# basilevh/tcow

Measured on AMD Instinct MI355X. Metric: train clips/sec (T=30, 240x320), higher is better.
Workload: dtype bf16; 1 GPU; TCOW Seeker train step: T=30 240x320 patch16, 12-layer divided space-time ViT (D=768), num_queries=3, causal_attention=1, 1 clip/GPU; clips_per_gpu=1, num_queries=3, parallelism=dp1, optimizer=AdamW lr 1e-4, clip 0.3

## Files before the change

### include/tcow_hip.h

```cpp
#ifndef TCOW_HIP_H
#define TCOW_HIP_H

#ifdef __cplusplus
extern "C" {
#endif

#define TCOW_OK 0
#define TCOW_ERR_INVALID_ARG (-1)
#define TCOW_ERR_LAUNCH (-2)
#define TCOW_ERR_UNSUPPORTED (-3)

#define TCOW_F32 0
#define TCOW_BF16 1
#define TCOW_F32X3 2

#define TCOW_ACT_NONE 0
#define TCOW_ACT_GELU 1
#define TCOW_ACT_DGELU 2
#define TCOW_ACT_GELU_DSAVE 3
#define TCOW_ACT_MUL_AUX 4

#define TCOW_ABI_VERSION 11
int tcow_version(void);
const char* tcow_last_error(void);

typedef struct {
    int M, N, K;
    int dtype;
    const void* A; long lda;
    const void* W; long ldw;
    void* C; long ldc; int out_f32;
    const float* bias;
    const float* row_scale;
    const float* resid; long ldr;
    int act;
    void* aux; long ldaux;
    int tile;
    const float* bias2;
    const float* row_scale2;
} tcow_gemm_args;
int tcow_gemm_nt(void* stream, const tcow_gemm_args* args);

int tcow_prof_gemm_begin(int max_launches);
int tcow_prof_gemm_end(double* total_ms, double* total_flops, long* launches);
int tcow_prof_attn_begin(int max_launches);
int tcow_prof_attn_end(double* ms4, double* flops4, double* bytes4, long* launches4);

long tcow_gemm_tn_workspace_bytes(int M, int N, int K);
int tcow_gemm_tn(void* stream, int dtype, int M, int N, int K, const void* dY, long ldy, const void* X,
                 long ldx, float* dW, long lddw, float* bias_grad, int accumulate, void* workspace,
                 long workspace_bytes);

typedef struct {
    int M, N, K;
    const void* dY; long ldy;
    const void* X; long ldx;
    float* dW; long lddw;
    float* bias_grad;
    int accumulate;
} tcow_tn_problem;
long tcow_gemm_tn_grouped_workspace_bytes(int dtype, int n, const tcow_tn_problem* problems);
int tcow_gemm_tn_grouped(void* stream, int dtype, int n, const tcow_tn_problem* problems, void* workspace, long workspace_bytes);
int tcow_gemm_tn_group_max(void);

typedef struct {
    int M, N, K;
    const float* A; long sai, sak;
    const float* B; long sbj, sbk;
    float* C; long ldc;
    int accumulate;
} tcow_sgemm;
int tcow_sgemm_x3_batched(void* stream, int n, const tcow_sgemm* problems);

int tcow_layernorm_fwd(void* stream, int dtype, int rows, int D, const float* x, long ldx, const float* gamma,
                       const float* beta, float eps, void* y, long ldy, float* mean, float* rstd);
long tcow_layernorm_bwd_workspace_bytes(int D);
int tcow_layernorm_bwd(void* stream, int dtype, int rows, int D, const void* dy, long lddy, const float* x, long ldx,
                       const float* mean, const float* rstd, const float* gamma, const float* dres, long lddres,
                       float* dx, long lddx, float* dgamma, float* dbeta, int accumulate, void* workspace,
                       long workspace_bytes, void* dx_cast, long lddx_cast, const float* cast_row_scale,
                       const float* colsum_row_scale, float* colsum_out);
typedef struct {
    const float* part; int parts, D;
    float* dgamma; float* dbeta; float* colsum_out;
    int accumulate;
} tcow_ln_fold_job;
int tcow_layernorm_bwd_parts(int rows, int with_colsum);
int tcow_layernorm_fold(void* stream, int n, const tcow_ln_fold_job* jobs);

typedef struct {
    int B, T, S;
    int D, heads;
    int causal;
    int dtype;
} tcow_attn_shape;
int tcow_attn_temporal_fwd(void* stream, const tcow_attn_shape* shape, const void* qkv, void* out, float* lse);
int tcow_attn_spatial_fwd(void* stream, const tcow_attn_shape* shape, const void* qkv, void* out, float* lse);
long tcow_attn_bwd_workspace_bytes(const tcow_attn_shape* shape);
int tcow_attn_temporal_bwd(void* stream, const tcow_attn_shape* shape, const void* qkv, const void* out,
                           const void* dout, const float* lse, void* dqkv, void* workspace, long workspace_bytes);
int tcow_attn_spatial_bwd(void* stream, const tcow_attn_shape* shape, const void* qkv, const void* out,
                          const void* dout, const float* lse, void* dqkv, void* workspace, long workspace_bytes);

#define TCOW_STREAM_MAX_FRAMES 1024
int tcow_attn_temporal_cached_fwd(void* stream, const tcow_attn_shape* chunk, int T_total, const int* t0_dev, const void* qkv, void* k_cache,
                                  void* v_cache, void* out);
int tcow_cls_stream(void* stream, int B, int c, int S, int D, float* x, float* cls_cache, const int* t0_dev);

int tcow_im2col(void* stream, int dtype, int B, int T, int H, int W, int P, const float* rgb, const float* query,
                int pretrained_norm, void* out);
int tcow_im2col_channels(void* stream, int dtype, int B, int T, int H, int W, int P, int C, const float* src,
                         int normalise, void* out);
int tcow_gather_frames(void* stream, int elem_bytes, int C, int Tv, int H, int W, int Tc, int h, int w, const void* src,
                       const int* frame_idx, const int* src_y, const int* src_x, void* out);
int tcow_resize_aa(void* stream, int C, int Tv, int H, int W, int Tc, int hc, int wc, int oh, int ow, const float* src, const int* frame_idx,
                   const int* ys, const int* xs, const int* ymin, const int* ysize, const float* wy, int ky, const int* xmin, const int* xsize,
                   const float* wx, int kx, float* out);

long tcow_photometric_workspace_bytes(int Tc);
int tcow_photometric(void* stream, int Tv, int H, int W, int Tc, int y0, int x0, int h, int w, const float* src, const int* frame_idx, int n_ops,
                     const int* ops, float brightness, float contrast, float saturation, float hue, int blur, const float* taps, int gray,
                     float* workspace, long workspace_bytes, float* out);

int tcow_embed_fwd(void* stream, int B, int T, int S, int D, float* x, const float* cls, const float* pos,
                   const float* time_embed);
int tcow_embed_bwd(void* stream, int B, int T, int S, int D, const float* g, float* dpos, float* dtime,
                   int accumulate);
int tcow_cls_merge(void* stream, int B, int T, int S, int D, float* x, int mode, int backward);
int tcow_cls_merge_bwd_cast(void* stream, int dtype, int B, int T, int S, int D, float* x, int mode, void* cast_out, long ldc,
                            const float* cast_scale);

int tcow_unpatchify_pool_fwd(void* stream, int dtype, int BT, int Hp, int Wp, int P, int C, int st, const void* pm,
                             float* pooled);
int tcow_unpatchify_pool_bwd(void* stream, int dtype, int BT, int Hp, int Wp, int P, int C, int st,
                             const float* dpooled, void* dpm);
int tcow_upsample_fwd(void* stream, int B, int T, int C, int h, int w, int st, int bilinear, const float* pooled,
                      float* out);
int tcow_upsample_bwd(void* stream, int B, int T, int C, int h, int w, int st, int bilinear, const float* dout,
                      float* dpooled);
#define TCOW_AMAX_SLOTS 64
int tcow_upsample_bwd_amax(void* stream, int B, int T, int C, int h, int w, int st, const float* dout, float* dpooled,
                           unsigned* amax_bits, int n_slots);
int tcow_flags_fwd(void* stream, int BT, int S, int D, int F, const float* x, const float* Wf, const float* bf,
                   float* flags);

int tcow_scale_unless_one(void* stream, float* x, long n, const float* scale);
int tcow_scale_cast(void* stream, int dtype, long rows, int D, const float* src, long ld_src, const float* row_scale,
                    void* dst, long ld_dst);
int tcow_droppath_rows(void* stream, int depth, int B, int T, int S, const float* u, const float* keep_p, const float* mask0, float* out);
int tcow_cast_transpose(void* stream, int dtype, int N, int K, const float* W, void* Wc, void* Wt);
long tcow_cast_desc_bytes(void);
int tcow_cast_transpose_batched(void* stream, int dtype, const void* table, int n, int total_tiles);

long tcow_adamw_chunk_bytes(void);
int tcow_adamw_clip_step(void* stream, const void* chunks, int n_chunks, float lr, float beta1, float beta2, float eps,
                         float weight_decay, int step, float max_norm, float* scratch);
int tcow_adamw_clip_step_scaled(void* stream, const void* chunks, int n_chunks, float lr, float beta1, float beta2, float eps,
                                float weight_decay, int step, float max_norm, float* scratch, const float* grad_inv_scale);
long tcow_adamw_tile_bytes(void);
int tcow_adamw_clip_step_cast(void* stream, const void* chunks, int n_chunks, const void* flat_chunks, int n_flat, const void* tiles, int n_tiles, float lr, float beta1,
                              float beta2, float eps, float weight_decay, int step, float max_norm, float* scratch, const float* grad_inv_scale);

typedef struct {
    long n_frames, frame_len, frames_per_seq;
    const float* logits;  long logits_seq_stride;
    const float* target;  long target_seq_stride;
    const float* pixel_w;
    const float* frame_w;
    int weighted_aot;
    float aot_loss;
    double topk_frac;
    float loss_weight;
    float* loss;
    float* total;
    float* dlogits;  long dlogits_seq_stride;
    void* ws;  size_t ws_bytes;
    int focal;
} tcow_mask_loss_args;
size_t tcow_mask_loss_workspace_bytes(long n_frames, long frame_len);
size_t tcow_mask_loss_workspace_bytes_for(long n_frames, long frame_len, double topk_frac, float aot_loss);
int tcow_mask_loss(void* stream, const tcow_mask_loss_args* args);
int tcow_mask_loss_batch(void* stream, const tcow_mask_loss_args* args, int n);

int tcow_iou_counts(void* stream, const float* logits, const float* target, long n_frames, long frame_len, int* counts);

int tcow_build_masks(void* stream, int B, int Q, int M, int T, long HW, int query_time, const unsigned char* segm,
                     const unsigned char* div_segm, const int* query_idx, const int* front_idx, const int* cont_idx,
                     float* query_mask, float* target_mask, unsigned char* snitch_occl_by_ptr, int* counts);

int tcow_build_query_masks(void* stream, int B, int Q, int K, int M, int T, long HW, int query_time, const unsigned char* segm,
                           const unsigned char* div_segm, const float* occl_fracs, const float* dag, const long long* sel, float front_thres,
                           float front_half_thres, float outer_thres, float occluded_weight, float zero_weight, float has_weight, int* idx_ws,
                           unsigned char* ids, float* flags, float* sel_occl_fracs, float* frame_w, float* query_mask, float* target_mask,
                           unsigned char* snitch_occl_by_ptr, int* counts);

int tcow_iou_means(void* stream, const int* counts, int n_seq, int C, int T, float* mean, int* count);

size_t tcow_snitch_weights_workspace_bytes(long n_frames, int H, int W);
int tcow_snitch_weights(void* stream, long n_seq, int T, int H, int W, const float* target_ch0, long target_seq_stride,
                        const unsigned char* snitch_occl_by_ptr, const float* frame_w, const int* pos_count, int class_balancing,
                        float hard_negative_factor, float* weights, void* ws, size_t ws_bytes);

#ifdef __cplusplus
}
#endif
#endif
```

### tcow_amd/_lib.py

```python
import ctypes
import os

_HERE = os.path.dirname(os.path.abspath(__file__))
LIB_PATH = os.environ.get('TCOW_LIB') or os.path.join(_HERE, 'libtcow_hip.so')
LIB_PATH_FP16 = os.path.join(_HERE, 'libtcow_hip_fp16.so')

TCOW_F32, TCOW_BF16, TCOW_F32X3 = 0, 1, 2
ACT_NONE, ACT_GELU, ACT_DGELU, ACT_GELU_DSAVE, ACT_MUL_AUX = 0, 1, 2, 3, 4


class TcowError(RuntimeError):
    """Raised when a libtcow_hip entry point returns a non-zero status (message from tcow_last_error)."""


class AttnShape(ctypes.Structure):
    _fields_ = [('B', ctypes.c_int), ('T', ctypes.c_int), ('S', ctypes.c_int), ('D', ctypes.c_int),
                ('heads', ctypes.c_int), ('causal', ctypes.c_int), ('dtype', ctypes.c_int)]


class GemmArgs(ctypes.Structure):
    _fields_ = [('M', ctypes.c_int), ('N', ctypes.c_int), ('K', ctypes.c_int), ('dtype', ctypes.c_int),
                ('A', ctypes.c_void_p), ('lda', ctypes.c_long), ('W', ctypes.c_void_p), ('ldw', ctypes.c_long),
                ('C', ctypes.c_void_p), ('ldc', ctypes.c_long), ('out_f32', ctypes.c_int),
                ('bias', ctypes.c_void_p), ('row_scale', ctypes.c_void_p), ('resid', ctypes.c_void_p),
                ('ldr', ctypes.c_long), ('act', ctypes.c_int), ('aux', ctypes.c_void_p), ('ldaux', ctypes.c_long), ('tile', ctypes.c_int),
                ('bias2', ctypes.c_void_p), ('row_scale2', ctypes.c_void_p)]


class SGemm(ctypes.Structure):
    _fields_ = [('M', ctypes.c_int), ('N', ctypes.c_int), ('K', ctypes.c_int),
                ('A', ctypes.c_void_p), ('sai', ctypes.c_long), ('sak', ctypes.c_long),
                ('B', ctypes.c_void_p), ('sbj', ctypes.c_long), ('sbk', ctypes.c_long),
                ('C', ctypes.c_void_p), ('ldc', ctypes.c_long), ('accumulate', ctypes.c_int)]


class TnProblem(ctypes.Structure):
    _fields_ = [('M', ctypes.c_int), ('N', ctypes.c_int), ('K', ctypes.c_int),
                ('dY', ctypes.c_void_p), ('ldy', ctypes.c_long), ('X', ctypes.c_void_p), ('ldx', ctypes.c_long),
                ('dW', ctypes.c_void_p), ('lddw', ctypes.c_long), ('bias_grad', ctypes.c_void_p), ('accumulate', ctypes.c_int)]


class LnFoldJob(ctypes.Structure):
    _fields_ = [('part', ctypes.c_void_p), ('parts', ctypes.c_int), ('D', ctypes.c_int), ('dgamma', ctypes.c_void_p), ('dbeta', ctypes.c_void_p),
                ('colsum_out', ctypes.c_void_p), ('accumulate', ctypes.c_int)]


class MaskLossArgs(ctypes.Structure):
    _fields_ = [('n_frames', ctypes.c_long), ('frame_len', ctypes.c_long), ('frames_per_seq', ctypes.c_long),
                ('logits', ctypes.c_void_p), ('logits_seq_stride', ctypes.c_long),
                ('target', ctypes.c_void_p), ('target_seq_stride', ctypes.c_long),
                ('pixel_w', ctypes.c_void_p), ('frame_w', ctypes.c_void_p),
                ('weighted_aot', ctypes.c_int), ('aot_loss', ctypes.c_float), ('topk_frac', ctypes.c_double),
                ('loss_weight', ctypes.c_float), ('loss', ctypes.c_void_p), ('total', ctypes.c_void_p),
                ('dlogits', ctypes.c_void_p), ('dlogits_seq_stride', ctypes.c_long),
                ('ws', ctypes.c_void_p), ('ws_bytes', ctypes.c_size_t), ('focal', ctypes.c_int)]


_libs = {}

_vp, _i, _l, _f = ctypes.c_void_p, ctypes.c_int, ctypes.c_long, ctypes.c_float
_ash = ctypes.POINTER(AttnShape)
SIGNATURES = {
    'tcow_version': (_i, []),
    'tcow_last_error': (ctypes.c_char_p, []),
    'tcow_gemm_nt': (_i, [_vp, ctypes.POINTER(GemmArgs)]),
    'tcow_prof_gemm_begin': (_i, [_i]),
    'tcow_prof_gemm_end': (_i, [ctypes.POINTER(ctypes.c_double), ctypes.POINTER(ctypes.c_double), ctypes.POINTER(ctypes.c_long)]),
    'tcow_prof_attn_begin': (_i, [_i]),
    'tcow_prof_attn_end': (_i, [_vp, _vp, _vp, _vp]),
    'tcow_gemm_tn_workspace_bytes': (_l, [_i, _i, _i]),
    'tcow_gemm_tn': (_i, [_vp, _i, _i, _i, _i, _vp, _l, _vp, _l, _vp, _l, _vp, _i, _vp, _l]),
    'tcow_gemm_tn_grouped_workspace_bytes': (_l, [_i, _i, _vp]),
    'tcow_gemm_tn_grouped': (_i, [_vp, _i, _i, _vp, _vp, _l]),
    'tcow_gemm_tn_group_max': (_i, []),
    'tcow_sgemm_x3_batched': (_i, [_vp, _i, _vp]),
    'tcow_layernorm_fwd': (_i, [_vp, _i, _i, _i, _vp, _l, _vp, _vp, _f, _vp, _l, _vp, _vp]),
    'tcow_layernorm_bwd_workspace_bytes': (_l, [_i]),
    'tcow_layernorm_bwd': (_i, [_vp, _i, _i, _i, _vp, _l, _vp, _l, _vp, _vp, _vp, _vp, _l, _vp, _l, _vp, _vp, _i, _vp, _l, _vp, _l, _vp, _vp, _vp]),
    'tcow_layernorm_bwd_parts': (_i, [_i, _i]),
    'tcow_layernorm_fold': (_i, [_vp, _i, _vp]),
    'tcow_attn_temporal_fwd': (_i, [_vp, _ash, _vp, _vp, _vp]),
    'tcow_attn_spatial_fwd': (_i, [_vp, _ash, _vp, _vp, _vp]),
    'tcow_attn_bwd_workspace_bytes': (_l, [_ash]),
    'tcow_attn_temporal_bwd': (_i, [_vp, _ash, _vp, _vp, _vp, _vp, _vp, _vp, _l]),
    'tcow_attn_spatial_bwd': (_i, [_vp, _ash, _vp, _vp, _vp, _vp, _vp, _vp, _l]),
    'tcow_attn_temporal_cached_fwd': (_i, [_vp, _ash, _i, _vp, _vp, _vp, _vp, _vp]),
    'tcow_cls_stream': (_i, [_vp, _i, _i, _i, _i, _vp, _vp, _vp]),
    'tcow_im2col': (_i, [_vp, _i, _i, _i, _i, _i, _i, _vp, _vp, _i, _vp]),
    'tcow_gather_frames': (_i, [_vp, _i, _i, _i, _i, _i, _i, _i, _i, _vp, _vp, _vp, _vp, _vp]),
    'tcow_resize_aa': (_i, [_vp, _i, _i, _i, _i, _i, _i, _i, _i, _i, _vp, _vp, _vp, _vp, _vp, _vp, _vp, _i, _vp, _vp, _vp, _i, _vp]),
    'tcow_photometric_workspace_bytes': (_l, [_i]),
    'tcow_photometric': (_i, [_vp, _i, _i, _i, _i, _i, _i, _i, _i, _vp, _vp, _i, ctypes.POINTER(ctypes.c_int), _f, _f, _f, _f, _i, ctypes.POINTER(ctypes.c_float), _i,
                         _vp, _l, _vp]),
    'tcow_im2col_channels': (_i, [_vp, _i, _i, _i, _i, _i, _i, _i, _vp, _i, _vp]),
    'tcow_embed_fwd': (_i, [_vp, _i, _i, _i, _i, _vp, _vp, _vp, _vp]),
    'tcow_embed_bwd': (_i, [_vp, _i, _i, _i, _i, _vp, _vp, _vp, _i]),
    'tcow_cls_merge': (_i, [_vp, _i, _i, _i, _i, _vp, _i, _i]),
    'tcow_cls_merge_bwd_cast': (_i, [_vp, _i, _i, _i, _i, _i, _vp, _i, _vp, _l, _vp]),
    'tcow_unpatchify_pool_fwd': (_i, [_vp, _i, _i, _i, _i, _i, _i, _i, _vp, _vp]),
    'tcow_unpatchify_pool_bwd': (_i, [_vp, _i, _i, _i, _i, _i, _i, _i, _vp, _vp]),
    'tcow_upsample_fwd': (_i, [_vp, _i, _i, _i, _i, _i, _i, _i, _vp, _vp]),
    'tcow_upsample_bwd': (_i, [_vp, _i, _i, _i, _i, _i, _i, _i, _vp, _vp]),
    'tcow_upsample_bwd_amax': (_i, [_vp, _i, _i, _i, _i, _i, _i, _vp, _vp, _vp, _i]),
    'tcow_flags_fwd': (_i, [_vp, _i, _i, _i, _i, _vp, _vp, _vp, _vp]),
    'tcow_droppath_rows': (_i, [_vp, _i, _i, _i, _i, _vp, _vp, _vp, _vp]),
    'tcow_scale_cast': (_i, [_vp, _i, _l, _i, _vp, _l, _vp, _vp, _l]),
    'tcow_scale_unless_one': (_i, [_vp, _vp, _l, _vp]),
    'tcow_cast_transpose': (_i, [_vp, _i, _i, _i, _vp, _vp, _vp]),
    'tcow_cast_desc_bytes': (_l, []),
    'tcow_cast_transpose_batched': (_i, [_vp, _i, _vp, _i, _i]),
    'tcow_adamw_chunk_bytes': (_l, []),
    'tcow_adamw_clip_step': (_i, [_vp, _vp, _i, _f, _f, _f, _f, _f, _i, _f, _vp]),
    'tcow_adamw_clip_step_scaled': (_i, [_vp, _vp, _i, _f, _f, _f, _f, _f, _i, _f, _vp, _vp]),
    'tcow_adamw_tile_bytes': (_l, []),
    'tcow_adamw_clip_step_cast': (_i, [_vp, _vp, _i, _vp, _i, _vp, _i, _f, _f, _f, _f, _f, _i, _f, _vp, _vp]),
    'tcow_mask_loss_workspace_bytes': (ctypes.c_size_t, [_l, _l]),
    'tcow_mask_loss_workspace_bytes_for': (ctypes.c_size_t, [_l, _l, ctypes.c_double, _f]),
    'tcow_mask_loss': (_i, [_vp, ctypes.POINTER(MaskLossArgs)]),
    'tcow_mask_loss_batch': (_i, [_vp, ctypes.POINTER(MaskLossArgs), _i]),
    'tcow_iou_counts': (_i, [_vp, _vp, _vp, _l, _l, _vp]),
    'tcow_build_masks': (_i, [_vp, _i, _i, _i, _i, _l, _i, _vp, _vp, _vp, _vp, _vp, _vp, _vp, _vp, _vp]),
    'tcow_build_query_masks': (_i, [_vp, _i, _i, _i, _i, _i, _l, _i, _vp, _vp, _vp, _vp, _vp, _f, _f, _f, _f, _f, _f, _vp, _vp, _vp, _vp, _vp, _vp, _vp, _vp, _vp]),
    'tcow_iou_means': (_i, [_vp, _vp, _i, _i, _i, _vp, _vp]),
    'tcow_snitch_weights_workspace_bytes': (ctypes.c_size_t, [_l, _i, _i]),
    'tcow_snitch_weights': (_i, [_vp, _l, _i, _i, _i, _vp, _l, _vp, _vp, _vp, _i, _f, _vp, _vp, ctypes.c_size_t]),
}


ABI_VERSION = 11


def _declare(L, tolerant=False):
    for name, (res, args) in SIGNATURES.items():
        if tolerant and not hasattr(L, name):
            continue
        fn = getattr(L, name)
        fn.restype = res
        fn.argtypes = args



def lib(fmt='bf16'):
    L = _libs.get(fmt)
    if L is None:
        path = LIB_PATH if fmt == 'bf16' else LIB_PATH_FP16
        if not os.path.exists(path):
            raise TcowError(f'{path} not found: build it with `make` (or __graft_entry__.build()); '
                            'the Seeker HIP path has no fallback')
        import torch
        L = ctypes.CDLL(path)
        L.tcow_last_error.restype = ctypes.c_char_p
        L.tcow_version.restype = ctypes.c_int
        if L.tcow_version() != ABI_VERSION and not (fmt == 'bf16' and os.environ.get('TCOW_LIB')):
            raise TcowError(f'{path} reports ABI version {L.tcow_version()}, this host code was written against {ABI_VERSION} (include/tcow_hip.h): rebuild with `make`')
        _declare(L, tolerant=(fmt == 'bf16' and bool(os.environ.get('TCOW_LIB'))))
        _libs[fmt] = L
    return L


def check(rc, what='', L=None):
    if rc != 0:
        raise TcowError(f'{what} failed (status {rc}): {(L or lib()).tcow_last_error().decode()}')
```

### tcow_amd/csrc/gemm_x3.hip

```cpp
#include "gemm_f32.h"

namespace {

constexpr int XT = 128;
constexpr int XK = 32;
constexpr int XP = 80;
constexpr int XPLANE = XT * XP;

typedef __attribute__((ext_vector_type(8))) __bf16 x3_bf16x8;
typedef __attribute__((ext_vector_type(2))) __bf16 x3_bf16x2;
__device__ __forceinline__ uint32_t x3_pack(float a, float b) {
    f32x2 v = {a, b};
    return __builtin_bit_cast(uint32_t, __builtin_convertvector(v, x3_bf16x2));
}
__device__ __forceinline__ void split2(float x0, float x1, uint32_t& h, uint32_t& l) {
    h = x3_pack(x0, x1);
    l = x3_pack(x0 - __builtin_bit_cast(float, h << 16), x1 - __builtin_bit_cast(float, h & 0xffff0000u));
}

enum { LD_ANY = 0, LD_KVEC = 1, LD_RVEC = 2 };

template <int LD>
__device__ __forceinline__ void load_regs(const float* __restrict__ P, long s_row, long s_k, int row0, int nrows, int k0, int K, f32x4 (&v)[4], int tid) {
    if (LD == LD_KVEC) {
        const int kq = k0 + (tid & 7) * 4, r = tid >> 3;
        const int kc = kq < K - 4 ? kq : K - 4;
#pragma unroll
        for (int ps = 0; ps < 4; ++ps) {
            int gr = row0 + r + 32 * ps; gr = gr < nrows ? gr : nrows - 1;
            v[ps] = *reinterpret_cast<const f32x4*>(P + (size_t)gr * s_row + kc);
        }
    } else if (LD == LD_RVEC) {
        const int rq = 4 * ((tid & 7) + 8 * (tid >> 6));
        int gr = row0 + rq; gr = gr < nrows - 4 ? gr : nrows - 4;
#pragma unroll
        for (int ps = 0; ps < 2; ++ps) {
            const int k = k0 + 2 * (((tid >> 3) & 7) + 8 * ps);
            const int kc0 = k < K ? k : K - 1, kc1 = k + 1 < K ? k + 1 : K - 1;
            v[2 * ps] = *reinterpret_cast<const f32x4*>(P + (size_t)kc0 * s_k + gr);
            v[2 * ps + 1] = *reinterpret_cast<const f32x4*>(P + (size_t)kc1 * s_k + gr);
        }
    } else {
        const int iq = tid & 31, kp = tid >> 5;
#pragma unroll
        for (int e = 0; e < 4; ++e) {
            int gr = row0 + iq + 32 * e; gr = gr < nrows ? gr : nrows - 1;
#pragma unroll
            for (int ps = 0; ps < 2; ++ps) {
                const int k = k0 + 2 * (kp + 8 * ps);
                const int kc0 = k < K ? k : K - 1, kc1 = k + 1 < K ? k + 1 : K - 1;
                v[e][2 * ps] = P[(size_t)gr * s_row + (size_t)kc0 * s_k];
                v[e][2 * ps + 1] = P[(size_t)gr * s_row + (size_t)kc1 * s_k];
            }
        }
    }
}

template <int LD>
__device__ __forceinline__ void mask_tail(f32x4 (&v)[4], int k0, int kend, int tid) {
    const f32x4 zero = {0.f, 0.f, 0.f, 0.f};
    if (LD == LD_KVEC) {
        const bool live = k0 + (tid & 7) * 4 < kend;
#pragma unroll
        for (int e = 0; e < 4; ++e) v[e] = live ? v[e] : zero;
    } else if (LD == LD_RVEC) {
#pragma unroll
        for (int ps = 0; ps < 2; ++ps) {
            const int k = k0 + 2 * (((tid >> 3) & 7) + 8 * ps);
            v[2 * ps] = k < kend ? v[2 * ps] : zero;
            v[2 * ps + 1] = k + 1 < kend ? v[2 * ps + 1] : zero;
        }
    } else {
#pragma unroll
        for (int e = 0; e < 4; ++e)
#pragma unroll
            for (int ps = 0; ps < 2; ++ps) {
                const int k = k0 + 2 * ((tid >> 5) + 8 * ps);
                v[e][2 * ps] = k < kend ? v[e][2 * ps] : 0.f; v[e][2 * ps + 1] = k + 1 < kend ? v[e][2 * ps + 1] : 0.f;
            }
    }
}

template <int LD>
__device__ __forceinline__ void store_split(const f32x4 (&v)[4], char* hi_plane, char* lo_plane, int tid) {
    if (LD == LD_KVEC) {
        const int kq = tid & 7, r = tid >> 3;
#pragma unroll
        for (int ps = 0; ps < 4; ++ps) {
            uint2 h, l;
            split2(v[ps][0], v[ps][1], h.x, l.x);
            split2(v[ps][2], v[ps][3], h.y, l.y);
            const int off = (r + 32 * ps) * XP + kq * 8;
            *reinterpret_cast<uint2*>(hi_plane + off) = h;
            *reinterpret_cast<uint2*>(lo_plane + off) = l;
        }
    } else if (LD == LD_RVEC) {
        const int rq = 4 * ((tid & 7) + 8 * (tid >> 6));
#pragma unroll
        for (int ps = 0; ps < 2; ++ps) {
            const int kp = ((tid >> 3) & 7) + 8 * ps;
#pragma unroll
            for (int e = 0; e < 4; ++e) {
                uint32_t h, l;
                split2(v[2 * ps][e], v[2 * ps + 1][e], h, l);
                const int off = (rq + e) * XP + kp * 4;
                *reinterpret_cast<uint32_t*>(hi_plane + off) = h;
                *reinterpret_cast<uint32_t*>(lo_plane + off) = l;
            }
        }
    } else {
        const int iq = tid & 31, kp = tid >> 5;
#pragma unroll
        for (int e = 0; e < 4; ++e)
#pragma unroll
            for (int ps = 0; ps < 2; ++ps) {
                uint32_t h, l;
                split2(v[e][2 * ps], v[e][2 * ps + 1], h, l);
                const int off = (iq + 32 * e) * XP + (kp + 8 * ps) * 4;
                *reinterpret_cast<uint32_t*>(hi_plane + off) = h;
                *reinterpret_cast<uint32_t*>(lo_plane + off) = l;
            }
    }
}

__device__ __forceinline__ int cdiv_dev(int a, int b) { return (a + b - 1) / b; }

__device__ __forceinline__ x3_bf16x8 frag(const char* plane, int row, int ks, int hi) {
    return __builtin_bit_cast(x3_bf16x8, *reinterpret_cast<const uint4*>(plane + row * XP + ks * 32 + hi * 16));
}

template <int LDA, int LDB>
__device__ __forceinline__ void gemm_x3_body(const F32Params& p, const int bid, const int kz, char* smem) {
    char* a_hi = smem; char* a_lo = smem + XPLANE; char* b_hi = smem + 2 * XPLANE; char* b_lo = smem + 3 * XPLANE;
    const int tid = threadIdx.x, lane = tid & 63, wave = tid >> 6;
    const int wm = wave >> 1, wn = wave & 1, l31 = lane & 31, hi = lane >> 5;
    const int tiles_n = cdiv_dev(p.N, XT), nblk = tiles_n * cdiv_dev(p.M, XT);
    const int q = nblk >> 3, rr = nblk & 7, xcd = bid & 7;
    const int pid = ((xcd < rr) ? xcd * (q + 1) : rr * (q + 1) + (xcd - rr) * q) + (bid >> 3);
    const int pm = pid / tiles_n;
    const int m0 = pm * XT, n0 = (pid - pm * tiles_n) * XT;
    const int kbeg = kz * p.kps;
    const int kend = (kbeg + p.kps < p.K) ? kbeg + p.kps : p.K;
    f32x16 acc[2][2];
#pragma unroll
    for (int i = 0; i < 2; ++i)
#pragma unroll
        for (int j = 0; j < 2; ++j)
#pragma unroll
            for (int r = 0; r < 16; ++r) acc[i][j][r] = 0.f;
    f32x4 ra0[4], rb0[4], ra1[4], rb1[4];
    auto fetch = [&](f32x4 (&ra)[4], f32x4 (&rb)[4], int k0) {
        load_regs<LDA>(p.A, p.sai, p.sak, m0, p.M, k0, p.K, ra, tid);
        load_regs<LDB>(p.B, p.sbj, p.sbk, n0, p.N, k0, p.K, rb, tid);
    };
    auto step = [&](f32x4 (&ra)[4], f32x4 (&rb)[4], int kcur, int knext) {
        if (kcur + XK > kend) { mask_tail<LDA>(ra, kcur, kend, tid); mask_tail<LDB>(rb, kcur, kend, tid); }
        store_split<LDA>(ra, a_hi, a_lo, tid);
        store_split<LDB>(rb, b_hi, b_lo, tid);
        __syncthreads();
        fetch(ra, rb, knext);
#pragma unroll
        for (int ks = 0; ks < 2; ++ks) {
            x3_bf16x8 ah[2], al[2], bh[2], bl[2];
#pragma unroll
            for (int i = 0; i < 2; ++i) {
                ah[i] = frag(a_hi, wm * 64 + i * 32 + l31, ks, hi); al[i] = frag(a_lo, wm * 64 + i * 32 + l31, ks, hi);
                bh[i] = frag(b_hi, wn * 64 + i * 32 + l31, ks, hi); bl[i] = frag(b_lo, wn * 64 + i * 32 + l31, ks, hi);
            }
#pragma unroll
            for (int i = 0; i < 2; ++i)
#pragma unroll
                for (int j = 0; j < 2; ++j) {
                    acc[i][j] = __builtin_amdgcn_mfma_f32_32x32x16_bf16(bh[j], al[i], acc[i][j], 0, 0, 0);
                    acc[i][j] = __builtin_amdgcn_mfma_f32_32x32x16_bf16(bl[j], ah[i], acc[i][j], 0, 0, 0);
                    acc[i][j] = __builtin_amdgcn_mfma_f32_32x32x16_bf16(bh[j], ah[i], acc[i][j], 0, 0, 0);
                }
        }
        __syncthreads();
    };
    fetch(ra0, rb0, kbeg);
    __builtin_amdgcn_sched_barrier(0);
    fetch(ra1, rb1, kbeg + XK);
    __builtin_amdgcn_sched_barrier(0);
    for (int k0 = kbeg; k0 < kend; k0 += 2 * XK) {
        step(ra0, rb0, k0, k0 + 2 * XK);
        step(ra1, rb1, k0 + XK, k0 + 3 * XK);
    }
    constexpr int CT_LD = 68;
    float* ct = reinterpret_cast<float*>(smem) + wave * (32 * CT_LD);
    const int c4 = (lane & 15) * 4, r4 = lane >> 4;
    const int gn = n0 + wn * 64 + c4;
    const bool v16 = p.slab ? ((reinterpret_cast<uintptr_t>(p.slab) & 15) == 0 && (p.N & 3) == 0)
                            : (((reinterpret_cast<uintptr_t>(p.C) | reinterpret_cast<uintptr_t>(p.resid) | reinterpret_cast<uintptr_t>(p.aux) | reinterpret_cast<uintptr_t>(p.bias2)) & 15) == 0 &&
                               ((p.ldc | p.ldr | p.ldaux) & 3) == 0);
    float4 b4 = make_float4(0.f, 0.f, 0.f, 0.f);
    if (!p.slab && p.bias) {
        if (gn < p.N) b4.x = p.bias[gn];
        if (gn + 1 < p.N) b4.y = p.bias[gn + 1];
        if (gn + 2 < p.N) b4.z = p.bias[gn + 2];
        if (gn + 3 < p.N) b4.w = p.bias[gn + 3];
    }
    float* slab = p.slab ? p.slab + (size_t)kz * p.M * p.N : nullptr;
#pragma unroll
    for (int i = 0; i < 2; ++i) {
#pragma unroll
        for (int j = 0; j < 2; ++j)
#pragma unroll
            for (int g = 0; g < 4; ++g)
                *reinterpret_cast<float4*>(ct + l31 * CT_LD + j * 32 + 8 * g + 4 * hi) = make_float4(acc[i][j][4 * g], acc[i][j][4 * g + 1], acc[i][j][4 * g + 2], acc[i][j][4 * g + 3]);
#pragma unroll 1
        for (int it = 0; it < 8; ++it) {
            const int row = it * 4 + r4;
            const int gm = m0 + wm * 64 + i * 32 + row;
            if (gm >= p.M || gn >= p.N) continue;
            const float4 x = *reinterpret_cast<const float4*>(ct + row * CT_LD + c4);
            if (v16 && gn + 3 < p.N) {
                if (slab) st4(slab + (size_t)gm * p.N + gn, x);
                else f32_epilogue_store4(p, gm, gn, x, b4);
            } else {
                const float xs[4] = {x.x, x.y, x.z, x.w}, bs[4] = {b4.x, b4.y, b4.z, b4.w};
                for (int e = 0; e < 4; ++e) {
                    if (gn + e >= p.N) break;
                    if (slab) slab[(size_t)gm * p.N + gn + e] = xs[e];
                    else f32_epilogue_store(p, gm, gn + e, xs[e], bs[e]);
                }
            }
        }
    }
}

template <int LD>
__global__ __launch_bounds__(256, LD == LD_ANY ? 2 : 3) void gemm_x3_kernel(F32Params p) {
    __shared__ __attribute__((aligned(16))) char smem[4 * XPLANE];
    gemm_x3_body<LD, LD>(p, blockIdx.x, blockIdx.y, smem);
}

constexpr int X3_MAX_BATCH = 24;
struct X3Batch { F32Params p[X3_MAX_BATCH]; };
template <int LDA, int LDB>
__global__ __launch_bounds__(256, (LDA == LD_ANY || LDB == LD_ANY) ? 2 : 3) void gemm_x3_batch_kernel(X3Batch b) {
    __shared__ __attribute__((aligned(16))) char smem[4 * XPLANE];
    const F32Params& p = b.p[blockIdx.y];
    if ((int)blockIdx.x >= cdiv_dev(p.N, XT) * cdiv_dev(p.M, XT)) return;
    gemm_x3_body<LDA, LDB>(p, blockIdx.x, 0, smem);
}

}

int tcow_launch_slab_reduce(hipStream_t stream, const float* slab, int nz, long slab_stride, long rows, long cols, float* out, long ldo, int accumulate,
                            const float* bias_part, int bias_nparts, int bias_n, float* bias_out);

int tcow_gemm_nt_x3(hipStream_t stream, const tcow_gemm_args* a) {
    F32Params p;
    p.M = a->M; p.N = a->N; p.K = a->K;
    p.A = (const float*)a->A; p.sai = a->lda; p.sak = 1;
    p.B = (const float*)a->W; p.sbj = a->ldw; p.sbk = 1;
    p.C = a->C; p.ldc = a->ldc; p.bias = a->bias; p.row_scale = a->row_scale; p.resid = a->resid; p.ldr = a->ldr;
    p.act = a->act; p.aux = (float*)a->aux; p.ldaux = a->ldaux; p.bias2 = a->bias2; p.row_scale2 = a->row_scale2; p.kps = ((a->K + XK - 1) / XK) * XK; p.slab = nullptr;
    const bool vec = ((reinterpret_cast<uintptr_t>(p.A) | reinterpret_cast<uintptr_t>(p.B)) & 15) == 0 && ((p.sai | p.sbj | p.K) & 3) == 0;
    const dim3 grid(cdiv(a->N, XT) * cdiv(a->M, XT), 1);
    if (vec) hipLaunchKernelGGL(gemm_x3_kernel<LD_KVEC>, grid, dim3(256), 0, stream, p);
    else hipLaunchKernelGGL(gemm_x3_kernel<LD_ANY>, grid, dim3(256), 0, stream, p);
    TCOW_CHECK_LAUNCH();
    return TCOW_OK;
}

int tcow_tn_splits_x3(int M, int N, int K) {
    const int tiles = cdiv(N, XT) * cdiv(K, XT);
    int s = (3 * 256) / tiles;
    const int max_s = M / 256;
    if (s > max_s) s = max_s;
    if (s > 64) s = 64;
    if (s < 1) s = 1;
    return s;
}

int tcow_gemm_tn_x3(hipStream_t stream, int M, int N, int K, const float* dY, long ldy, const float* X, long ldx, float* dW, long lddw,
                    int accumulate, float* slab, int splits, const float* bias_part, int bias_nparts, float* bias_out) {
    F32Params p;
    p.M = N; p.N = K; p.K = M;
    p.A = dY; p.sai = 1; p.sak = ldy;
    p.B = X; p.sbj = 1; p.sbk = ldx;
    p.C = nullptr; p.ldc = 0; p.bias = nullptr; p.row_scale = nullptr; p.resid = nullptr; p.ldr = 0; p.act = 0; p.aux = nullptr; p.ldaux = 0; p.bias2 = nullptr; p.row_scale2 = nullptr;
    int kps = cdiv(M, splits); kps = ((kps + XK - 1) / XK) * XK;
    const int nz = cdiv(M, kps);
    p.kps = kps; p.slab = slab;
    const bool vec = ((reinterpret_cast<uintptr_t>(dY) | reinterpret_cast<uintptr_t>(X)) & 15) == 0 && ((ldy | ldx | N | K) & 3) == 0;
    const dim3 grid(cdiv(K, XT) * cdiv(N, XT), nz);
    if (vec) hipLaunchKernelGGL(gemm_x3_kernel<LD_RVEC>, grid, dim3(256), 0, stream, p);
    else hipLaunchKernelGGL(gemm_x3_kernel<LD_ANY>, grid, dim3(256), 0, stream, p);
    TCOW_CHECK_LAUNCH();
    return tcow_launch_slab_reduce(stream, slab, nz, (long)N * K, N, K, dW, lddw, accumulate, bias_part, bias_nparts, N, bias_out);
}

static int x3_loader(const float* P, long s_row, long s_k, int nrows, int K) {
    const bool al = (reinterpret_cast<uintptr_t>(P) & 15) == 0;
    if (s_k == 1 && al && (s_row & 3) == 0 && (K & 3) == 0 && K >= 4) return LD_KVEC;
    if (s_row == 1 && al && (s_k & 3) == 0 && (nrows & 3) == 0 && nrows >= 4) return LD_RVEC;
    return LD_ANY;
}

extern "C" int tcow_sgemm_x3_batched(void* stream, int n, const tcow_sgemm* probs) {
    TCOW_CHECK_ARG(n >= 1 && n <= X3_MAX_BATCH && probs, "tcow_sgemm_x3_batched: 1 .. %d problems per call (got %d)", X3_MAX_BATCH, n);
    X3Batch b;
    int lda = -1, ldb = -1, maxtiles = 0;
    for (int i = 0; i < n; ++i) {
        const tcow_sgemm& s = probs[i];
        TCOW_CHECK_ARG(s.M > 0 && s.N > 0 && s.K > 0 && s.A && s.B && s.C && s.ldc >= s.N, "tcow_sgemm_x3_batched: bad problem %d", i);
        F32Params& p = b.p[i];
        p.M = s.M; p.N = s.N; p.K = s.K; p.A = s.A; p.sai = s.sai; p.sak = s.sak; p.B = s.B; p.sbj = s.sbj; p.sbk = s.sbk;
        p.C = s.C; p.ldc = s.ldc; p.bias = nullptr; p.row_scale = nullptr; p.resid = nullptr; p.ldr = 0; p.act = 0; p.aux = nullptr; p.ldaux = 0; p.bias2 = nullptr; p.row_scale2 = nullptr;
        p.kps = ((s.K + XK - 1) / XK) * XK; p.slab = nullptr;
        if (s.accumulate) { p.resid = s.C; p.ldr = s.ldc; }
        const int la = x3_loader(s.A, s.sai, s.sak, s.M, s.K), lb = x3_loader(s.B, s.sbj, s.sbk, s.N, s.K);
        lda = (lda < 0 || lda == la) ? la : LD_ANY; ldb = (ldb < 0 || ldb == lb) ? lb : LD_ANY;
        const int t = cdiv(s.N, XT) * cdiv(s.M, XT);
        if (t > maxtiles) maxtiles = t;
    }
    const dim3 grid(maxtiles, n);
    hipStream_t st = (hipStream_t)stream;
    if (lda == LD_KVEC && ldb == LD_KVEC) hipLaunchKernelGGL((gemm_x3_batch_kernel<LD_KVEC, LD_KVEC>), grid, dim3(256), 0, st, b);
    else if (lda == LD_KVEC && ldb == LD_RVEC) hipLaunchKernelGGL((gemm_x3_batch_kernel<LD_KVEC, LD_RVEC>), grid, dim3(256), 0, st, b);
    else if (lda == LD_RVEC && ldb == LD_RVEC) hipLaunchKernelGGL((gemm_x3_batch_kernel<LD_RVEC, LD_RVEC>), grid, dim3(256), 0, st, b);
    else if (lda == LD_RVEC && ldb == LD_ANY) hipLaunchKernelGGL((gemm_x3_batch_kernel<LD_RVEC, LD_ANY>), grid, dim3(256), 0, st, b);
    else hipLaunchKernelGGL((gemm_x3_batch_kernel<LD_ANY, LD_ANY>), grid, dim3(256), 0, st, b);
    TCOW_CHECK_LAUNCH();
    return TCOW_OK;
}
```

### tcow_amd/csrc/optim.hip

```cpp
#include "common.h"

namespace {

struct Chunk { float* p; const float* g; float* m; float* v; long n; };

__global__ __launch_bounds__(256) void sumsq_kernel(const Chunk* __restrict__ chunks, float* __restrict__ partial) {
    __shared__ float red[4];
    const Chunk c = chunks[blockIdx.x];
    float s = 0.f;
    const long n4 = c.n >> 2;
    for (long i = threadIdx.x; i < n4; i += 256) { const float4 g = ld4(c.g + i * 4); s += g.x * g.x + g.y * g.y + g.z * g.z + g.w * g.w; }
    for (long i = (n4 << 2) + threadIdx.x; i < c.n; i += 256) s += c.g[i] * c.g[i];
    s = wave_sum(s);
    if ((threadIdx.x & 63) == 0) red[threadIdx.x >> 6] = s;
    __syncthreads();
    if (threadIdx.x == 0) partial[blockIdx.x] = (red[0] + red[1]) + (red[2] + red[3]);
}

__global__ __launch_bounds__(256) void clipcoef_kernel(const float* __restrict__ partial, int n, float max_norm, float* __restrict__ out ,
                                                       const float* __restrict__ gscale) {
    __shared__ float red[4];
    float s = 0.f;
    for (int i = threadIdx.x; i < n; i += 256) s += partial[i];
    s = wave_sum(s);
    if ((threadIdx.x & 63) == 0) red[threadIdx.x >> 6] = s;
    __syncthreads();
    if (threadIdx.x == 0) {
        const float gs = gscale ? gscale[0] : 1.0f;
        const float norm = sqrtf((red[0] + red[1]) + (red[2] + red[3])) * gs;
        float coef = max_norm > 0.f ? max_norm / (norm + 1e-6f) : 1.0f;
        const bool skip = !(norm <= 3.0e38f);
        out[0] = skip ? -1.0f : (coef < 1.0f ? coef : 1.0f) * gs;
        out[1] = norm;
        if (skip) out[2] += 1.0f;
    }
}

__global__ __launch_bounds__(256) void adamw_kernel(const Chunk* __restrict__ chunks, const float* __restrict__ coef_ptr, float lr, float beta1, float beta2, float eps,
                                                    float weight_decay, int step) {
    const Chunk c = chunks[blockIdx.x];
    const float coef = coef_ptr[0];
    if (coef < 0.f) return;
    const float eff = fmaxf((float)step - coef_ptr[2], 1.0f);
    const float bc1 = 1.0f - powf(beta1, eff), bc2_sqrt = sqrtf(1.0f - powf(beta2, eff));
    const float decay = 1.0f - lr * weight_decay, step_size = lr / bc1;
    const long n4 = c.n >> 2;
    auto upd = [&](float& p, float g, float& m, float& v) {
        g *= coef;
        p *= decay;
        m = beta1 * m + (1.0f - beta1) * g;
        v = beta2 * v + (1.0f - beta2) * g * g;
        p -= step_size * m / (sqrtf(v) / bc2_sqrt + eps);
    };
    for (long i = threadIdx.x; i < n4; i += 256) {
        float4 p = ld4(c.p + i * 4), m = ld4(c.m + i * 4), v = ld4(c.v + i * 4);
        const float4 g = ld4(c.g + i * 4);
        upd(p.x, g.x, m.x, v.x); upd(p.y, g.y, m.y, v.y); upd(p.z, g.z, m.z, v.z); upd(p.w, g.w, m.w, v.w);
        st4(c.p + i * 4, p); st4(c.m + i * 4, m); st4(c.v + i * 4, v);
    }
    for (long i = (n4 << 2) + threadIdx.x; i < c.n; i += 256) upd(c.p[i], c.g[i], c.m[i], c.v[i]);
}

struct CastTile { float* p; const float* g; float* m; float* v; bf16_t* wc; bf16_t* wt; int K, N; };

__global__ __launch_bounds__(256) void adamw_cast_kernel(const CastTile* __restrict__ tiles, const float* __restrict__ coef_ptr, float lr, float beta1, float beta2, float eps,
                                                         float weight_decay, int step) {
    __shared__ float tile[64][65];
    const float coef = coef_ptr[0];
    if (coef < 0.f) return;
    const CastTile d = tiles[blockIdx.x];
    const float eff = fmaxf((float)step - coef_ptr[2], 1.0f);
    const float bc1 = 1.0f - powf(beta1, eff), bc2_sqrt = sqrtf(1.0f - powf(beta2, eff));
    const float decay = 1.0f - lr * weight_decay, step_size = lr / bc1;
    auto upd = [&](float& p, float g, float& m, float& v) {
        g *= coef;
        p *= decay;
        m = beta1 * m + (1.0f - beta1) * g;
        v = beta2 * v + (1.0f - beta2) * g * g;
        p -= step_size * m / (sqrtf(v) / bc2_sqrt + eps);
    };
    const int c4 = (threadIdx.x & 15) * 4, r0 = threadIdx.x >> 4;
#pragma unroll
    for (int i = 0; i < 4; ++i) {
        const int r = r0 + 16 * i;
        const size_t o = (size_t)r * d.K + c4;
        float4 p = ld4(d.p + o), m = ld4(d.m + o), v = ld4(d.v + o);
        const float4 g = ld4(d.g + o);
        upd(p.x, g.x, m.x, v.x); upd(p.y, g.y, m.y, v.y); upd(p.z, g.z, m.z, v.z); upd(p.w, g.w, m.w, v.w);
        st4(d.p + o, p); st4(d.m + o, m); st4(d.v + o, v);
        st4(d.wc + o, p);
        tile[r][c4] = p.x; tile[r][c4 + 1] = p.y; tile[r][c4 + 2] = p.z; tile[r][c4 + 3] = p.w;
    }
    __syncthreads();
#pragma unroll
    for (int i = 0; i < 4; ++i) {
        const int k = r0 + 16 * i;
        st4(d.wt + (size_t)k * d.N + c4, make_float4(tile[c4][k], tile[c4 + 1][k], tile[c4 + 2][k], tile[c4 + 3][k]));
    }
}

}

extern "C" {

long tcow_adamw_chunk_bytes(void) { return (long)sizeof(Chunk); }
long tcow_adamw_tile_bytes(void) { return (long)sizeof(CastTile); }

int tcow_adamw_clip_step_cast(void* stream, const void* chunks, int n_chunks, const void* flat_chunks, int n_flat, const void* tiles, int n_tiles, float lr, float beta1,
                              float beta2, float eps, float weight_decay, int step, float max_norm, float* scratch, const float* grad_inv_scale) {
    TCOW_CHECK_ARG(chunks && scratch && n_chunks > 0 && step >= 1 && n_flat >= 0 && (flat_chunks || n_flat == 0) && n_tiles >= 0 && (tiles || n_tiles == 0),
                   "tcow_adamw_clip_step_cast: bad arguments");
    const Chunk* c = (const Chunk*)chunks;
    hipLaunchKernelGGL(sumsq_kernel, dim3(n_chunks), dim3(256), 0, (hipStream_t)stream, c, scratch);
    TCOW_CHECK_LAUNCH();
    hipLaunchKernelGGL(clipcoef_kernel, dim3(1), dim3(256), 0, (hipStream_t)stream, scratch, n_chunks, max_norm, scratch + n_chunks, grad_inv_scale);
    TCOW_CHECK_LAUNCH();
    if (n_flat > 0) {
        hipLaunchKernelGGL(adamw_kernel, dim3(n_flat), dim3(256), 0, (hipStream_t)stream, (const Chunk*)flat_chunks, scratch + n_chunks, lr, beta1, beta2, eps, weight_decay, step);
        TCOW_CHECK_LAUNCH();
    }
    if (n_tiles > 0) {
        hipLaunchKernelGGL(adamw_cast_kernel, dim3(n_tiles), dim3(256), 0, (hipStream_t)stream, (const CastTile*)tiles, scratch + n_chunks, lr, beta1, beta2, eps, weight_decay, step);
        TCOW_CHECK_LAUNCH();
    }
    return TCOW_OK;
}

int tcow_adamw_clip_step_scaled(void* stream, const void* chunks, int n_chunks, float lr, float beta1, float beta2, float eps, float weight_decay, int step,
                                float max_norm, float* scratch, const float* grad_inv_scale) {
    TCOW_CHECK_ARG(chunks && scratch && n_chunks > 0 && step >= 1, "tcow_adamw_clip_step: bad arguments");
    const Chunk* c = (const Chunk*)chunks;
    hipLaunchKernelGGL(sumsq_kernel, dim3(n_chunks), dim3(256), 0, (hipStream_t)stream, c, scratch);
    TCOW_CHECK_LAUNCH();
    hipLaunchKernelGGL(clipcoef_kernel, dim3(1), dim3(256), 0, (hipStream_t)stream, scratch, n_chunks, max_norm, scratch + n_chunks, grad_inv_scale);
    TCOW_CHECK_LAUNCH();
    hipLaunchKernelGGL(adamw_kernel, dim3(n_chunks), dim3(256), 0, (hipStream_t)stream, c, scratch + n_chunks, lr, beta1, beta2, eps, weight_decay, step);
    TCOW_CHECK_LAUNCH();
    return TCOW_OK;
}

int tcow_adamw_clip_step(void* stream, const void* chunks, int n_chunks, float lr, float beta1, float beta2, float eps, float weight_decay, int step,
                         float max_norm, float* scratch) {
    return tcow_adamw_clip_step_scaled(stream, chunks, n_chunks, lr, beta1, beta2, eps, weight_decay, step, max_norm, scratch, nullptr);
}

}
```

### tcow_amd/engine.py

```python
import os
import torch

from . import ops
from .ops import ACT_GELU, ACT_GELU_DSAVE, ACT_MUL_AUX

def _layout(module):
    if module.attention_type == 'divided_space_time':
        return 20, dict(tn=0, tqkv=2, tproj=4, tfc=6, n1=8, qkv=10, proj=12, n2=14, fc1=16, fc2=18)
    return 12, dict(n1=0, qkv=2, proj=4, n2=6, fc1=8, fc2=10)


def _joint_rows(module, g, dev):
    key = ('jrows', g['B'], str(dev))
    idx = module._wcache.get(key)
    if idx is None:
        B, T, S = g['B'], g['T'], g['S']
        r = torch.arange(B * T * S, device=dev).reshape(B, T * S)
        keep = torch.ones(T * S, dtype=torch.bool, device=dev)
        keep[torch.arange(1, T, device=dev) * S] = False
        idx = r[:, keep].reshape(-1).contiguous()
        module._wcache[key] = idx
    return idx


def _w2d(p):
    return p.reshape(p.shape[0], -1)


def _get_weight(module, p, train):
    mode = module.mode
    key = id(p)
    ent = module._wcache.get(key)
    ver = (p._version, getattr(module, '_wepoch', 0))
    if ent is not None and ent[0] == ver and ent[1] == mode and (ent[3] is not None or not train):
        return ent[2], ent[3]
    w = _w2d(p.detach())
    N, K = w.shape
    dt = ops.tdtype(mode)
    if ops.is16(mode):
        Wc = torch.empty(N, K, dtype=dt, device=w.device)
        Wt = torch.empty(K, N, dtype=dt, device=w.device) if train else None
        ops.cast_transpose(mode, w.contiguous(), Wc, Wt)
    else:
        Wc = w.contiguous()
        Wt = None
        if train:
            Wt = torch.empty(K, N, dtype=dt, device=w.device)
            ops.cast_transpose(mode, Wc, None, Wt)
    module._wcache[key] = (ver, mode, Wc, Wt)
    if train:
        reg = module.__dict__.setdefault('_wreg', {})
        reg[key] = (p, Wc if ops.is16(mode) else None, Wt, N, K)
        module.__dict__['_wreg_gen'] = module.__dict__.get('_wreg_gen', 0) + 1
    return Wc, Wt


def group_sizes(depth, spec=None):
    if spec is None:
        spec = os.environ.get('TCOW_DDP_GROUP') or ('5,5,2' if depth == 12 else '4')
    want = [max(1, int(x)) for x in str(spec).split(',') if x.strip()] or [4]
    sizes, left, k = [], depth, 0
    while left > 0:
        gs = min(want[min(k, len(want) - 1)], left)
        sizes.append(gs); left -= gs; k += 1
    return sizes


def _fold_on(module):
    return ops.is16(module.mode) and module.attention_type == 'divided_space_time'


def _fold_products(ents):
    for c0 in range(0, len(ents), 24):
        ops.sgemm_batched([(e['fc'].detach(), e['proj'].detach(), e['W32']) for e in ents[c0:c0 + 24]])
        ops.sgemm_batched([(e['fc'].detach(), e['bproj'].detach().view(1, -1).t(), e['b32'].view(-1, 1)) for e in ents[c0:c0 + 24]])


def _folded_weight(module, i, q, ix, train):
    pfc, pproj, bproj = q[ix['tfc']], q[ix['tproj']], q[ix['tproj'] + 1]
    key = ('fold', i)
    ver = (pfc._version, pproj._version, bproj._version, getattr(module, '_wepoch', 0))
    ent = module._wcache.get(key)
    if ent is not None and ent['ver'] == ver and ent['mode'] == module.mode and (ent['Wt'] is not None or not train):
        return ent['Wc'], ent['Wt'], ent['b32']
    D = pfc.shape[0]
    dev = pfc.device
    dt = ops.tdtype(module.mode)
    if ent is None or ent['mode'] != module.mode:
        ent = dict(fc=pfc, proj=pproj, bproj=bproj, W32=torch.empty(D, D, dtype=torch.float32, device=dev), b32=torch.empty(D, dtype=torch.float32, device=dev),
                   Wc=torch.empty(D, D, dtype=dt, device=dev), Wt=None, mode=module.mode)
    if train and ent['Wt'] is None:
        ent['Wt'] = torch.empty(D, D, dtype=dt, device=dev)
    _fold_products([ent])
    ops.cast_transpose(module.mode, ent['W32'], ent['Wc'], ent['Wt'])
    ent['ver'] = ver
    module._wcache[key] = ent
    if train:
        module.__dict__.setdefault('_wreg', {})[key] = (ent['W32'], ent['Wc'], ent['Wt'], D, D)
        module.__dict__.setdefault('_foldreg', {})[key] = ent
    return ent['Wc'], ent['Wt'], ent['b32']


def refresh_weights(module):
    import struct
    reg = getattr(module, '_wreg', None)
    if not reg:
        return False
    mode = module.mode
    folds = module.__dict__.get('_foldreg')
    if folds:
        live = [ent for k, ent in folds.items() if k in reg]
        if live:
            _fold_products(live)
    done = module.__dict__.pop('_opt_cast_keys', None) or ()
    all_ents = list(reg.items())
    ents = [(k, v) for k, v in all_ents if k not in done]
    if not ents:
        _stamp_versions(module, all_ents, folds, mode)
        return True
    sig = tuple((k, p.data_ptr(), 0 if Wc is None else Wc.data_ptr(), 0 if Wt is None else Wt.data_ptr()) for k, (p, Wc, Wt, N, K) in ents) + (mode,)
    tab = module.__dict__.get('_wtab')
    if tab is None or tab[0] != sig:
        rec, tiles = [], 0
        edge = 64 if all(N % 64 == 0 and K % 64 == 0 for _, (_, _, _, N, K) in ents) else 32
        for k, (p, Wc, Wt, N, K) in ents:
            rec.append(struct.pack('<QQQiiii', p.data_ptr(), 0 if Wc is None else Wc.data_ptr(), 0 if Wt is None else Wt.data_ptr(), N, K, tiles, edge))
            tiles += ((N + edge - 1) // edge) * ((K + edge - 1) // edge)
        assert len(rec[0]) == L_cast_desc_bytes()
        dev = ents[0][1][0].device
        buf = torch.frombuffer(bytearray(b''.join(rec)), dtype=torch.uint8).to(dev)
        tab = (sig, buf, len(rec), tiles)
        module.__dict__['_wtab'] = tab
    ops.cast_transpose_batched(mode, tab[1], tab[2], tab[3])
    _stamp_versions(module, all_ents, folds, mode)
    return True


def _stamp_versions(module, ents, folds, mode):
    epoch = getattr(module, '_wepoch', 0)
    for k, (p, Wc, Wt, N, K) in ents:
        if folds and k in folds:
            e = folds[k]
            e['ver'] = (e['fc']._version, e['proj']._version, e['bproj']._version, epoch)
            continue
        w = _w2d(p.detach())
        module._wcache[k] = ((p._version, epoch), mode, Wc if Wc is not None else w.contiguous(), Wt)


def L_cast_desc_bytes():
    from . import _lib
    return int(_lib.lib().tcow_cast_desc_bytes())


def _row_vectors(module, g, train):
    B, T, S, N = g['B'], g['T'], g['S'], g['N']
    dev = module.vit.pos_embed.device
    key = ('mask0', B, T, str(dev))
    mask0 = module._wcache.get(key)
    if mask0 is None:
        mask0 = torch.ones(B, T, S, dtype=torch.float32, device=dev)
        mask0[:, :, 0] = 0
        mask0 = mask0.reshape(-1).contiguous()
        module._wcache[key] = mask0
    depth = module.network_depth
    rates = torch.linspace(0, module.drop_path_rate, depth).tolist() if depth > 1 else [0.0]
    scales = []
    forced = module.forced_drop_masks
    joint = module.attention_type != 'divided_space_time'
    if joint:
        for i in range(depth):
            ent = {'t': None, 's': None, 'm': None}
            for kind, name in (('s', 'spatial'), ('m', 'mlp')):
                if forced is not None:
                    if (i, name) in forced:
                        keep, rate = forced[(i, name)]
                        ent[kind] = (keep.to(dev, torch.float32).reshape(B) / (1.0 - rate))[:, None].expand(B, T * S).reshape(-1).contiguous()
                elif train and rates[i] > 0.:
                    keep = (torch.rand(B, device=dev) + (1.0 - rates[i])).floor_()
                    ent[kind] = (keep / (1.0 - rates[i]))[:, None].expand(B, T * S).reshape(-1).contiguous()
            scales.append(ent)
        return mask0, scales
    if forced is None and train and max(rates) > 0.:
        kkey = ('keep_p', tuple(rates), str(dev))
        keep_p = module._wcache.get(kkey)
        if keep_p is None:
            keep_p = (1.0 - torch.tensor(rates, dtype=torch.float32)).to(dev)
            module._wcache[kkey] = keep_p
        u = torch.rand(depth, B * N + B * T + B, device=dev)
        if u.is_cuda and N == S - 1:
            from . import ops
            rt, rsp, rml, rt0 = ops.droppath_rows(u, keep_p, mask0, B, T, S)
        else:
            kp = keep_p[:, None]
            sc = (u + kp).floor_() / kp
            kt = sc[:, :B * N].reshape(depth, B, 1, N); ks = sc[:, B * N:B * N + B * T].reshape(depth, B, T, 1); km = sc[:, B * N + B * T:].reshape(depth, B, 1)
            rt = torch.ones(depth, B, T, S, dtype=torch.float32, device=dev)
            rt[:, :, :, 1:] = kt
            rt = rt.reshape(depth, -1)
            rsp = ks.expand(depth, B, T, S).reshape(depth, -1)
            rml = km.expand(depth, B, T * S).reshape(depth, -1)
            rt0 = rt * mask0[None, :]
        for i in range(depth):
            live = rates[i] > 0.
            scales.append({'t': rt[i] if live else None, 's': rsp[i] if live else None, 'm': rml[i] if live else None, 't0': rt0[i] if live else mask0})
        return mask0, scales
    for i in range(depth):
        r = rates[i]
        ent = {'t': None, 's': None, 'm': None}
        if forced is not None or (train and r > 0.):
            def draw(kind, shape):
                if forced is not None:
                    if (i, kind) not in forced:
                        return None
                    keep, rate = forced[(i, kind)]
                    return keep.to(dev, torch.float32).reshape(shape) / (1.0 - rate)
                keep = (torch.rand(shape, device=dev) + (1.0 - r)).floor_()
                return keep / (1.0 - r)
            kt = draw('temporal', (B, N))
            if kt is not None:
                rs = torch.ones(B, T, S, dtype=torch.float32, device=dev)
                rs[:, :, 1:] = kt[:, None, :]
                ent['t'] = rs.reshape(-1).contiguous()
            ks = draw('spatial', (B, T))
            if ks is not None:
                ent['s'] = ks[:, :, None].expand(B, T, S).reshape(-1).contiguous()
            km = draw('mlp', (B,))
            if km is not None:
                ent['m'] = km[:, None].expand(B, T * S).reshape(-1).contiguous()
        ent['t0'] = mask0 if ent['t'] is None else ent['t'] * mask0
        scales.append(ent)
    return mask0, scales


def _effective_embeddings(module, g):
    v = module.vit
    pos = v.pos_embed.detach()[0]
    S, T = g['S'], g['T']
    pos_idx = None
    if pos.shape[0] != S:
        n_old = pos.shape[0] - 1
        Pold = int(n_old ** 0.5)
        Hn = S // g['Wp']
        ys = (torch.arange(Hn, device=pos.device).float() * (Pold / Hn)).floor().long().clamp_(max=Pold - 1)
        xs = (torch.arange(g['Wp'], device=pos.device).float() * (Pold / g['Wp'])).floor().long().clamp_(max=Pold - 1)
        grid = (ys[:, None] * Pold + xs[None, :]).reshape(-1) + 1
        pos_idx = torch.cat([torch.zeros(1, dtype=torch.long, device=pos.device), grid])
        pos = pos[pos_idx].contiguous()
    te = v.time_embed.detach()[0]
    time_idx = None
    if te.shape[0] != T:
        time_idx = (torch.arange(T, device=te.device).float() * (te.shape[0] / T)).floor().long().clamp_(max=te.shape[0] - 1)
        te = te[time_idx].contiguous()
    return pos.contiguous(), te.contiguous(), pos_idx, time_idx


def run_forward(module, rgb, qm, params, save, stream=None):
    mode = module.mode
    gmode = module.gemm_mode
    dt = ops.tdtype(mode)
    dev = rgb.device
    B = qm.shape[0]
    g = module.geometry(B) if stream is None else module.geometry(B, T=rgb.shape[2])
    T, S, D, M, P, heads = g['T'], g['S'], g['D'], g['M'], g['P'], g['heads']
    ca = module.causal_attention
    use_cls = ca in (0, 1)
    train = save
    f32 = torch.float32

    def E(*shape, dtype=dt):
        return torch.empty(*shape, dtype=dtype, device=dev)

    W = lambda p: _get_weight(module, p, train)[0]
    mask0, dps = _row_vectors(module, g, module.training)
    sv = {'g': g, 'blocks': [], 'mask0': mask0, 'dps': dps} if save else None

    Kpe = module.input_channels * P * P
    X = E(M, D, dtype=f32)
    Bc = rgb.shape[0]
    Qs = B // Bc
    if Qs > 1:
        Krgb = 3 * P * P
        Wc = W(params[3])
        A_rgb = E(Bc * T * S, Krgb); A_m = E(M, Kpe - Krgb)
        ops.im2col_channels(mode, rgb, P, module.tracker_pretrained, A_rgb)
        ops.im2col_channels(mode, qm, P, False, A_m)
        Xrgb = E(Bc * T * S, D, dtype=f32)
        ops.gemm_nt(gmode, A_rgb, Wc[:, :Krgb], Xrgb, bias=params[4].detach())
        TS = T * S
        for bq in range(B):
            b = bq // Qs
            ops.gemm_nt(gmode, A_m[bq * TS:(bq + 1) * TS], Wc[:, Krgb:], X[bq * TS:(bq + 1) * TS], resid=Xrgb[b * TS:(b + 1) * TS])
        A_pe = (A_rgb, A_m)
    else:
        A_pe = E(M, Kpe)
        ops.im2col(mode, rgb, qm, P, module.tracker_pretrained, A_pe)
        ops.gemm_nt(gmode, A_pe, W(params[3]), X, bias=params[4].detach())
    if stream is None:
        pos, te, pos_idx, time_idx = _effective_embeddings(module, g)
    else:
        pos, te, pos_idx, time_idx = stream.pos, stream.time_rows, None, None
    ops.embed_fwd(X, B, T, S, params[0].detach().reshape(-1), pos, te)
    if save:
        sv.update(A_pe=A_pe, pos_idx=pos_idx, time_idx=time_idx)

    BP, ix = _layout(module)
    joint = module.attention_type != 'divided_space_time'
    fold = _fold_on(module)
    amode = gmode if gmode == ops.F32X3 else mode
    shape_attn = ops.attn_shape(amode, B, T, S, D, heads, ca)
    if joint:
        jrows = _joint_rows(module, g, dev)
        Lj = 1 + T * (S - 1)
        shape_joint = ops.attn_shape(amode, B, 1, Lj, D, heads, 0)
    for i in range(module.network_depth):
        q = params[5 + i * BP: 5 + (i + 1) * BP]
        P_ = lambda name, k=0: q[ix[name] + k].detach()
        n1_w, n1_b, qkv_b, proj_b, n2_w, n2_b, fc1_w, fc1_b, fc2_b = P_('n1'), P_('n1', 1), P_('qkv', 1), P_('proj', 1), P_('n2'), P_('n2', 1), P_('fc1'), P_('fc1', 1), P_('fc2', 1)
        dp = dps[i]
        st = {}
        R0 = X
        if joint:
            V = E(M, D); mu1 = E(M, dtype=f32) if save else None; rs1 = E(M, dtype=f32) if save else None
            ops.layernorm_fwd(mode, R0, n1_w, n1_b, V, mu1, rs1)
            QKV2 = E(M, 3 * D)
            ops.gemm_nt(gmode, V, W(q[ix['qkv']]), QKV2, bias=qkv_b)
            QJ = QKV2.index_select(0, jrows)
            OJ = E(B * Lj, D); lse_s = E(B * Lj, heads, dtype=f32) if save else None
            ops.attn_fwd(shape_joint, True, QJ, OJ, lse_s)
            O2 = torch.zeros(M, D, dtype=dt, device=dev)
            O2.index_copy_(0, jrows, OJ)
            rs_s = dp['s']
            R2 = E(M, D, dtype=f32) if save else R0
            ops.gemm_nt(gmode, O2, W(q[ix['proj']]), R2, bias=proj_b, row_scale=rs_s, resid=R0)
            if save:
                st.update(R1=R0, mu1=mu1, rs1=rs1, V=V, QKV_s=QJ, O_s=O2, OJ=OJ, lse_s=lse_s, rs_s=rs_s)
        else:
            tn_w, tn_b, tqkv_b, tproj_b, tfc_b = P_('tn'), P_('tn', 1), P_('tqkv', 1), P_('tproj', 1), P_('tfc', 1)
            U = E(M, D); mu0 = E(M, dtype=f32) if save else None; rs0 = E(M, dtype=f32) if save else None
            ops.layernorm_fwd(mode, R0, tn_w, tn_b, U, mu0, rs0)
            QKV = E(M, 3 * D)
            ops.gemm_nt(gmode, U, W(q[ix['tqkv']]), QKV, bias=tqkv_b)
            O = E(M, D); lse_t = E(M, heads, dtype=f32) if save else None
            if stream is None:
                ops.attn_fwd(shape_attn, False, QKV, O, lse_t)
            else:
                ops.attn_temporal_cached(amode, B, T, S, D, heads, ca, stream.T_total, stream.t0_dev, QKV, stream.k_cache[i], stream.v_cache[i], O)
            R1 = E(M, D, dtype=f32) if save else R0
            if fold:
                Wf, _, bprime = _folded_weight(module, i, q, ix, train)
                ops.gemm_nt(gmode, O, Wf, R1, bias=bprime, row_scale=dp['t0'], resid=R0, bias2=tfc_b, row_scale2=mask0)
                Pj = None
            else:
                Pj = E(M, D)
                ops.gemm_nt(gmode, O, W(q[ix['tproj']]), Pj, bias=tproj_b, row_scale=dp['t'])
                ops.gemm_nt(gmode, Pj, W(q[ix['tfc']]), R1, bias=tfc_b, row_scale=mask0, resid=R0)
            if save:
                st.update(R0=R0, mu0=mu0, rs0=rs0, U=U, QKV_t=QKV, O_t=O, lse_t=lse_t, Pj=Pj)
            V = E(M, D); mu1 = E(M, dtype=f32) if save else None; rs1 = E(M, dtype=f32) if save else None
            ops.layernorm_fwd(mode, R1, n1_w, n1_b, V, mu1, rs1)
            QKV2 = E(M, 3 * D)
            ops.gemm_nt(gmode, V, W(q[ix['qkv']]), QKV2, bias=qkv_b)
            O2 = E(M, D); lse_s = E(M, heads, dtype=f32) if save else None
            ops.attn_fwd(shape_attn, True, QKV2, O2, lse_s)
            rs_s = dp['s']
            if not use_cls:
                rs_s = mask0 if rs_s is None else rs_s * mask0
            R2 = E(M, D, dtype=f32) if save else R1
            ops.gemm_nt(gmode, O2, W(q[ix['proj']]), R2, bias=proj_b, row_scale=rs_s, resid=R1)
            if use_cls and stream is not None:
                ops.cls_stream(R2, B, T, S, stream.cls_cache[i], stream.t0_dev)
            elif use_cls:
                ops.cls_merge(R2, B, T, S, 1 if ca == 1 else 0)
            if save:
                st.update(R1=R1, mu1=mu1, rs1=rs1, V=V, QKV_s=QKV2, O_s=O2, lse_s=lse_s, rs_s=rs_s)
        Wn = E(M, D); mu2 = E(M, dtype=f32) if save else None; rs2 = E(M, dtype=f32) if save else None
        ops.layernorm_fwd(mode, R2, n2_w, n2_b, Wn, mu2, rs2)
        Hd = fc1_w.shape[0]
        pre = E(M, Hd) if save else None
        H = E(M, Hd)
        ops.gemm_nt(gmode, Wn, W(q[ix['fc1']]), H, bias=fc1_b, act=ACT_GELU_DSAVE if save else ACT_GELU, aux=pre)
        R3 = E(M, D, dtype=f32) if save else R2
        ops.gemm_nt(gmode, H, W(q[ix['fc2']]), R3, bias=fc2_b, row_scale=dp['m'], resid=R2)
        if save:
            st.update(R2=R2, mu2=mu2, rs2=rs2, Wn=Wn, pre=pre, H=H)
            sv['blocks'].append(st)
        X = R3

    nb = 5 + module.network_depth * BP
    norm_w, norm_b, head_w, head_b = params[nb], params[nb + 1], params[nb + 2], params[nb + 3]
    feat32 = X
    if module.norm_embeddings:
        Fm = E(M, D); muf = E(M, dtype=f32) if save else None; rsf = E(M, dtype=f32) if save else None
        ops.layernorm_fwd(mode, X, norm_w.detach(), norm_b.detach(), Fm, muf, rsf)
        if module.flag_channels > 0 and mode != ops.F32:
            feat32 = E(M, D, dtype=f32)
            ops.layernorm_fwd(ops.F32, X, norm_w.detach(), norm_b.detach(), feat32)
        elif mode == ops.F32:
            feat32 = Fm
        if save:
            sv.update(muf=muf, rsf=rsf)
    elif mode == ops.F32:
        Fm = X
    else:
        Fm = E(M, D)
        ops.scale_cast(mode, X, None, Fm)
    Co = module.output_channels
    Pm = E(M, Co * P * P)
    ops.gemm_nt(gmode, Fm, W(head_w), Pm, bias=head_b.detach())
    stp = module.track_map_stride if module.track_map_stride > 1 else 1
    h, w = module.frame_height // stp, module.frame_width // stp
    pooled = E(B * T, Co, h, w, dtype=f32)
    ops.unpatchify_pool_fwd(mode, Pm, B * T, g['Hp'], g['Wp'], P, Co, stp, pooled)
    out_mask = E(B, Co, T, module.frame_height, module.frame_width, dtype=f32)
    bilinear = (module.track_map_resize == 'bilinear') and stp > 1
    ops.upsample_fwd(pooled, B, T, Co, h, w, stp, bilinear, out_mask)
    if module.flag_channels > 0:
        flags = E(B, T, module.flag_channels, dtype=f32)
        ops.flags_fwd(feat32, B * T, S, params[nb + 4].detach(), params[nb + 5].detach(), flags)
    else:
        flags = torch.zeros(0, device=dev)
    if save:
        sv.update(X_final=X, Fm=Fm, feat32=feat32, stp=stp, bilinear=bilinear, h=h, w=w)
    return out_mask, flags, sv


def run_backward(module, sv, params, d_mask, d_flags):
    mode = module.mode
    gmode = module.gemm_mode
    dt = ops.tdtype(mode)
    g = sv['g']
    B, T, S, D, M, P, heads = g['B'], g['T'], g['S'], g['D'], g['M'], g['P'], g['heads']
    dev = sv['X_final'].device
    ca = module.causal_attention
    use_cls = ca in (0, 1)
    f32 = torch.float32
    mask0 = sv['mask0']
    gscale = inv_gscale = None
    ls_mode = getattr(module, 'loss_scale', 'dynamic') if mode == ops.FP16 else None
    if ls_mode == 'dynamic' and _live_optim(module) is None and not module.__dict__.get('_warned_ls'):
        import warnings
        module.__dict__['_warned_ls'] = True
        warnings.warn("precision='fp16' with the dynamic loss scale but no FusedAdamWClip(..., module=net) attached: nothing lowers the scale "
                      "after an overflow or skips the poisoned step -- pass module= to the optimizer or set net.seeker.loss_scale to a number")

    def choose_scale(mask_amax):
        if ls_mode is None:
            return None, None
        if ls_mode == 'dynamic':
            amax = mask_amax if mask_amax is not None else torch.zeros((), dtype=f32, device=dev)
            if d_flags is not None and d_flags.numel():
                amax = torch.maximum(amax, d_flags.detach().abs().amax().to(f32))
            gs = torch.exp2(torch.floor(module.ls_log2 - torch.log2(amax.clamp_min(1e-37)))).clamp(2.0 ** -20, 2.0 ** 60)
        elif float(ls_mode) != 1.0:
            gs = torch.tensor(float(ls_mode), dtype=f32, device=dev)
        else:
            return None, None
        return gs, 1.0 / gs

    def E(*shape, dtype=dt):
        return torch.empty(*shape, dtype=dtype, device=dev)

    Wt = lambda p: _get_weight(module, p, True)[1]
    grads = [None] * len(params)

    defer_unscale = ((module.grad_hook is None or getattr(module.grad_hook, 'active', True) is False) and _live_optim(module) is not None
                     and bool(getattr(module, 'persistent_grads', False)) and not getattr(module, '_is_replica', False)
                     and module.__dict__.get('_defer_unscale', True))

    def publish(tag, flat):
        if inv_gscale is not None and not defer_unscale:
            flat.mul_(inv_gscale)
        if module.grad_hook is not None:
            module.grad_hook(tag, flat)

    def bucket(indices):
        indices = list(indices)
        total = sum(params[j].numel() for j in indices)
        flat = None
        if getattr(module, 'persistent_grads', False):
            key = ('gbuf', indices[0], total, str(dev))
            flat = module._gbufs.get(key)
            if flat is None:
                flat = module._gbufs[key] = torch.empty(total, dtype=f32, device=dev)
        if flat is None:
            flat = torch.empty(total, dtype=f32, device=dev)
        off = 0
        for j in indices:
            n = params[j].numel()
            grads[j] = flat[off:off + n].view(params[j].shape)
            off += n
        return flat

    def galloc(idx):
        return grads[idx]

    pending = []

    def linear_bwd(idx_w, dY, Xin, defer=False):
        dW = galloc(idx_w); db = galloc(idx_w + 1)
        if defer:
            pending.append((dY, Xin, dW.reshape(dW.shape[0], -1), db))
        else:
            ops.gemm_tn(gmode, dY, Xin, dW.reshape(dW.shape[0], -1), bias_grad=db)

    tn_group_max = ops.tn_group_max()

    ln_jobs = []

    def flush_pending():
        if pending:
            ops.gemm_tn_grouped(gmode, pending)
            pending.clear()
        if ln_jobs:
            ops.layernorm_fold(ln_jobs)

    BP, ix = _layout(module)
    joint = module.attention_type != 'divided_space_time'
    fold = _fold_on(module)
    depth = module.network_depth
    nb = 5 + depth * BP
    Co = module.output_channels
    have_flags = module.flag_channels > 0 and d_flags is not None and d_flags.numel() > 0
    head_idx = ([nb, nb + 1] if module.norm_embeddings else []) + [nb + 2, nb + 3] + ([nb + 4, nb + 5] if have_flags else [])
    group_lo = {}
    hi_ = depth
    for gs in group_sizes(depth):
        for j in range(hi_ - gs, hi_):
            group_lo[j] = hi_ - gs
        hi_ -= gs
    top_lo = group_lo[depth - 1]
    late = set()
    if fold:
        for j in range(depth):
            late.update((5 + j * BP + ix['tproj'], 5 + j * BP + ix['tproj'] + 1, 5 + j * BP + ix['tfc']))
    late_flat = bucket(sorted(late)) if late else None
    blk_idx = lambda lo_, hi_: [j for j in range(5 + lo_ * BP, 5 + hi_ * BP) if j not in late]
    flat_cur = bucket((list(range(0, 5)) if top_lo == 0 else []) + blk_idx(top_lo, depth) + head_idx)
    fold_jobs = []

    def fold_tmp(i):
        t = module._gbufs.get(('foldtmp', i, str(dev)))
        if t is None:
            t = module._gbufs[('foldtmp', i, str(dev))] = (torch.empty(D, D, dtype=f32, device=dev), torch.empty(D, dtype=f32, device=dev))
        return t

    def finish_fold_group():
        if not fold_jobs:
            return
        nt_, r1_, tn_, gv_ = [], [], [], []
        for (i, tW, tb) in fold_jobs:
            o_ = 5 + i * BP
            wfc, wp, bp = params[o_ + ix['tfc']].detach(), params[o_ + ix['tproj']].detach(), params[o_ + ix['tproj'] + 1].detach()
            nt_.append((tW, wp.t(), grads[o_ + ix['tfc']]))
            r1_.append((tb.view(-1, 1), bp.view(1, -1), grads[o_ + ix['tfc']]))
            tn_.append((wfc.t(), tW, grads[o_ + ix['tproj']]))
            gv_.append((wfc.t(), tb.view(-1, 1), grads[o_ + ix['tproj'] + 1].view(-1, 1)))
        for c0 in range(0, len(nt_), 24):
            ops.sgemm_batched(nt_[c0:c0 + 24]); ops.sgemm_batched(r1_[c0:c0 + 24], accumulate=True)
            ops.sgemm_batched(tn_[c0:c0 + 24]); ops.sgemm_batched(gv_[c0:c0 + 24])
        fold_jobs.clear()

    if d_mask is None:
        d_mask = torch.zeros(B, Co, T, module.frame_height, module.frame_width, dtype=f32, device=dev)
    d_mask = d_mask.to(f32).contiguous()
    dpooled = E(B * T, Co, sv['h'], sv['w'], dtype=f32)
    mask_amax = None
    if ls_mode == 'dynamic' and sv['bilinear'] and sv['stp'] == 4 and sv['h'] > 4 and sv['w'] > 4:
        _, mask_amax = ops.upsample_bwd_amax(d_mask, B, T, Co, sv['h'], sv['w'], sv['stp'], dpooled)
    else:
        if ls_mode == 'dynamic' and d_mask.numel():
            mask_amax = d_mask.abs().amax()
        ops.upsample_bwd(d_mask, B, T, Co, sv['h'], sv['w'], sv['stp'], sv['bilinear'], dpooled)
    gscale, inv_gscale = choose_scale(mask_amax)
    if gscale is not None:
        dpooled.mul_(gscale)
        d_flags = None if d_flags is None else d_flags * gscale
    dPm = E(M, Co * P * P)
    ops.unpatchify_pool_bwd(mode, dpooled, B * T, g['Hp'], g['Wp'], P, Co, sv['stp'], dPm)
    linear_bwd(nb + 2, dPm, sv['Fm'])
    dFeat = E(M, D, dtype=f32)
    ops.gemm_nt(gmode, dPm, Wt(params[nb + 2]), dFeat)
    if module.flag_channels > 0 and have_flags:
        df = d_flags.to(f32).reshape(B * T, -1).contiguous()
        meanf = sv['feat32'].reshape(B * T, S, D)[:, 1:, :].float().mean(dim=1)
        dmean = torch.empty(B * T, D, dtype=f32, device=dev)
        ops.sgemm_batched([(df.t(), meanf, grads[nb + 4])])
        ops.sgemm_batched([(df, params[nb + 4].detach(), dmean)])
        grads[nb + 5].copy_(df.sum(0))
        dFeat.reshape(B * T, S, D)[:, 1:, :] += (dmean / float(S - 1))[:, None, :]
    if module.norm_embeddings:
        dX = E(M, D, dtype=f32)
        ops.layernorm_bwd(ops.F32, dFeat, sv['X_final'], sv['muf'], sv['rsf'], params[nb].detach(), None, dX, galloc(nb), galloc(nb + 1))
    else:
        dX = dFeat
    amode = gmode if gmode == ops.F32X3 else mode
    shape_attn = ops.attn_shape(amode, B, T, S, D, heads, ca)
    if joint:
        jrows = _joint_rows(module, g, dev)
        Lj = 1 + T * (S - 1)
        shape_joint = ops.attn_shape(amode, B, 1, Lj, D, heads, 0)
    dR3 = dX
    G3_next = None
    for i in reversed(range(module.network_depth)):
        o = 5 + i * BP
        q = params[o: o + BP]
        st = sv['blocks'][i]
        dp = sv['dps'][i]
        Hd = q[ix['fc1']].shape[0]
        if i != depth - 1 and group_lo[i] != group_lo[i + 1]:
            lo_ = group_lo[i]
            flat_cur = bucket((list(range(0, 5)) if lo_ == 0 else []) + blk_idx(lo_, i + 1))
        next_scale = (sv['dps'][i - 1]['m'] if i > 0 else mask0)
        if G3_next is not None:
            G3 = G3_next
        else:
            G3 = E(M, D)
            ops.scale_cast(mode, dR3, dp['m'], G3)
        dpre = E(M, Hd)
        ops.gemm_nt(gmode, G3, Wt(q[ix['fc2']]), dpre, act=ACT_MUL_AUX, aux=st['pre'])
        linear_bwd(o + ix['fc2'], G3, st['H'], defer=True)
        dWn = E(M, D)
        ops.gemm_nt(gmode, dpre, Wt(q[ix['fc1']]), dWn)
        linear_bwd(o + ix['fc1'], dpre, st['Wn'], defer=True)
        dR2 = E(M, D, dtype=f32)
        G2 = E(M, D)
        ops.layernorm_bwd(mode, dWn, st['R2'], st['mu2'], st['rs2'], q[ix['n2']].detach(), dR3, dR2, galloc(o + ix['n2']), galloc(o + ix['n2'] + 1),
                          dx_cast=G2, cast_scale=st['rs_s'], defer=ln_jobs)
        del G3, dpre, dWn
        if use_cls and not joint:
            ops.cls_merge(dR2, B, T, S, 1 if ca == 1 else 0, backward=True, cast_mode=mode, cast_out=G2, cast_scale=st['rs_s'])
        dO2 = E(M, D)
        ops.gemm_nt(gmode, G2, Wt(q[ix['proj']]), dO2)
        linear_bwd(o + ix['proj'], G2, st['O_s'], defer=True)
        if joint:
            dQJ = E(B * Lj, 3 * D)
            ops.attn_bwd(shape_joint, True, st['QKV_s'], st['OJ'], dO2.index_select(0, jrows), st['lse_s'], dQJ)
            dQKV2 = torch.zeros(M, 3 * D, dtype=dt, device=dev)
            dQKV2.index_copy_(0, jrows, dQJ)
        else:
            dQKV2 = E(M, 3 * D)
            ops.attn_bwd(shape_attn, True, st['QKV_s'], st['O_s'], dO2, st['lse_s'], dQKV2)
        dV = E(M, D)
        ops.gemm_nt(gmode, dQKV2, Wt(q[ix['qkv']]), dV)
        linear_bwd(o + ix['qkv'], dQKV2, st['V'], defer=True)
        dR1 = E(M, D, dtype=f32)
        G1 = E(M, D)
        if fold:
            ops.layernorm_bwd(mode, dV, st['R1'], st['mu1'], st['rs1'], q[ix['n1']].detach(), dR2, dR1, galloc(o + ix['n1']), galloc(o + ix['n1'] + 1), dx_cast=G1,
                              cast_scale=dp['t0'], colsum_out=galloc(o + ix['tfc'] + 1), colsum_scale=mask0, defer=ln_jobs)
        else:
            ops.layernorm_bwd(mode, dV, st['R1'], st['mu1'], st['rs1'], q[ix['n1']].detach(), dR2, dR1, galloc(o + ix['n1']), galloc(o + ix['n1'] + 1), dx_cast=G1,
                              cast_scale=(next_scale if joint else mask0), defer=ln_jobs)
        del G2, dO2, dQKV2, dV
        if joint:
            G3_next = G1
            dR3 = dR1
        else:
            dO = E(M, D)
            if fold:
                ops.gemm_nt(gmode, G1, _folded_weight(module, i, q, ix, True)[1], dO)
                tW, tb = fold_tmp(i)
                pending.append((G1, st['O_t'], tW, tb))
                fold_jobs.append((i, tW, tb))
            else:
                dPj = E(M, D)
                ops.gemm_nt(gmode, G1, Wt(q[ix['tfc']]), dPj, row_scale=dp['t'])
                linear_bwd(o + ix['tfc'], G1, st['Pj'], defer=True)
                ops.gemm_nt(gmode, dPj, Wt(q[ix['tproj']]), dO)
                linear_bwd(o + ix['tproj'], dPj, st['O_t'], defer=True)
            dQKV = E(M, 3 * D)
            ops.attn_bwd(shape_attn, False, st['QKV_t'], st['O_t'], dO, st['lse_t'], dQKV)
            dU = E(M, D)
            ops.gemm_nt(gmode, dQKV, Wt(q[ix['tqkv']]), dU)
            linear_bwd(o + ix['tqkv'], dQKV, st['U'], defer=True)
            dR0 = E(M, D, dtype=f32)
            G3_next = E(M, D)
            ops.layernorm_bwd(mode, dU, st['R0'], st['mu0'], st['rs0'], q[ix['tn']].detach(), dR1, dR0, galloc(o + ix['tn']), galloc(o + ix['tn'] + 1),
                              dx_cast=G3_next, cast_scale=next_scale, defer=ln_jobs)
            dR3 = dR0
        if group_lo[i] == i or len(pending) + 8 > tn_group_max:
            flush_pending()
        sv['blocks'][i] = None
        if i > 0 and group_lo[i] == i:
            publish('g%d' % i, flat_cur)

    gX = dR3
    finish_fold_group()
    if late_flat is not None:
        publish('fold', late_flat)
    resized = sv['pos_idx'] is not None or sv['time_idx'] is not None
    dpos_eff = grads[1][0] if sv['pos_idx'] is None else E(S, D, dtype=f32)
    dtime_eff = grads[2][0] if sv['time_idx'] is None else E(T, D, dtype=f32)
    ops.embed_bwd(gX, B, T, S, dpos_eff, dtime_eff)
    grads[0].copy_(dpos_eff[0].reshape(1, 1, D))
    if sv['pos_idx'] is not None:
        grads[1].zero_()
        grads[1][0].index_add_(0, sv['pos_idx'], dpos_eff)
    if sv['time_idx'] is not None:
        grads[2].zero_()
        grads[2][0].index_add_(0, sv['time_idx'], dtime_eff)
    if G3_next is not None:
        Gpe = G3_next
    else:
        Gpe = E(M, D)
        ops.scale_cast(mode, gX, mask0, Gpe)
    dWpe = galloc(3).reshape(D, -1)
    if isinstance(sv['A_pe'], tuple):
        A_rgb, A_m = sv['A_pe']
        Krgb = A_rgb.shape[1]
        Bc = A_rgb.shape[0] // (T * S)
        Gsum = E(Bc * T * S, D)
        ops.scale_cast(mode, gX.reshape(Bc, B // Bc, T * S, D).sum(dim=1).reshape(Bc * T * S, D), mask0[:Bc * T * S], Gsum)
        ops.gemm_tn(gmode, Gsum, A_rgb, dWpe[:, :Krgb])
        ops.gemm_tn(gmode, Gpe, A_m, dWpe[:, Krgb:])
    else:
        ops.gemm_tn(gmode, Gpe, sv['A_pe'], dWpe)
    grads[4].copy_(dtime_eff.sum(0))
    publish('g0', flat_cur)
    module.__dict__['pending_inv_scale'] = inv_gscale if defer_unscale else None
    if module.grad_hook is not None:
        if hasattr(module.grad_hook, 'finish'):
            module.grad_hook.finish()
    return grads


def _live_optim(module):
    ref = module.__dict__.get('_optim_ref')
    return ref() if ref is not None else None


class SeekerFunction(torch.autograd.Function):

    @staticmethod
    def forward(ctx, module, rgb, qm, *params):
        need = any(ctx.needs_input_grad[3:])
        ctx.set_materialize_grads(False)
        out_mask, flags, sv = run_forward(module, rgb, qm, params, save=need)
        ctx.module = module
        ctx.sv = sv
        ctx.params = params
        return out_mask, flags

    @staticmethod
    def backward(ctx, d_mask, d_flags):
        if ctx.sv is None:
            raise ops.L.TcowError('backward called on a forward that did not save activations')
        grads = run_backward(ctx.module, ctx.sv, ctx.params, d_mask, d_flags)
        ctx.sv = None
        out = []
        persistent = getattr(ctx.module, 'persistent_grads', False)
        for p, gr, need in zip(ctx.params, grads, ctx.needs_input_grad[3:]):
            if not need or gr is None:
                out.append(None)
                continue
            gr = gr.reshape(p.shape)
            if persistent and (p.grad is None or p.grad.data_ptr() == gr.data_ptr()):
                p.grad = gr
                out.append(None)
            else:
                out.append(gr)
        return (None, None, None, *out)
```

### tcow_amd/ops.py

```python
import ctypes
import threading

import numpy as np
import torch

from . import _lib as L

F32, BF16 = L.TCOW_F32, L.TCOW_BF16
F32X3 = L.TCOW_F32X3
ACT_NONE, ACT_GELU, ACT_DGELU, ACT_GELU_DSAVE, ACT_MUL_AUX = L.ACT_NONE, L.ACT_GELU, L.ACT_DGELU, L.ACT_GELU_DSAVE, L.ACT_MUL_AUX


FP16 = 16


def tdtype(mode):
    return torch.bfloat16 if mode == BF16 else torch.float16 if mode == FP16 else torch.float32


def is16(mode):
    return mode in (BF16, FP16)


def _sel(mode):
    return (L.lib('fp16'), BF16) if mode == FP16 else (L.lib(), mode)


_raw_stream = getattr(torch._C, '_cuda_getCurrentRawStream', None)
_cur_device = getattr(torch._C, '_cuda_getDevice', None)


def _stream():
    if _raw_stream is not None and _cur_device is not None:
        return _raw_stream(_cur_device())
    return torch.cuda.current_stream().cuda_stream


def _p(t):
    return t.data_ptr() if t is not None else None


def _need_cuda(*ts):
    for t in ts:
        if t is not None and not t.is_cuda:
            raise L.TcowError('libtcow_hip kernels need CUDA/HIP tensors (no CPU fallback on this path)')


def gemm_nt(mode, A, W, out, bias=None, row_scale=None, resid=None, act=ACT_NONE, aux=None, tile=0, bias2=None, row_scale2=None):
    _need_cuda(A, W, out)
    M, K = A.shape
    N = W.shape[0]
    lib, dm = _sel(mode)
    a = L.GemmArgs(M, N, K, dm, A.data_ptr(), A.stride(0), W.data_ptr(), W.stride(0), out.data_ptr(), out.stride(0),
                   1 if out.dtype == torch.float32 else 0, _p(bias), _p(row_scale), _p(resid),
                   resid.stride(0) if resid is not None else 0, act, _p(aux), aux.stride(0) if aux is not None else 0, int(tile), _p(bias2), _p(row_scale2))
    L.check(lib.tcow_gemm_nt(_stream(), ctypes.byref(a)), 'tcow_gemm_nt', lib)
    return out


_ws_cache = {}


def workspace(nbytes, device, tag='default'):
    key = (str(device), _stream(), tag, threading.get_ident())
    buf = _ws_cache.get(key)
    if buf is None or buf.numel() < nbytes:
        if buf is None and len(_ws_cache) >= 48:
            alive = {t.ident for t in threading.enumerate()}
            for k in [k for k in _ws_cache if k[3] not in alive]:
                del _ws_cache[k]
        buf = torch.empty(int(nbytes * 1.25) + 1024, dtype=torch.uint8, device=device)
        _ws_cache[key] = buf
    return buf


def gemm_tn(mode, dY, X, dW, bias_grad=None, accumulate=False):
    _need_cuda(dY, X, dW)
    M, N = dY.shape
    K = X.shape[1]
    lib, dm = _sel(mode)
    nbytes = lib.tcow_gemm_tn_workspace_bytes(M, N, K)
    ws = workspace(nbytes, dY.device, 'tn')
    L.check(lib.tcow_gemm_tn(_stream(), dm, M, N, K, dY.data_ptr(), dY.stride(0), X.data_ptr(), X.stride(0), dW.data_ptr(),
                             dW.stride(0), _p(bias_grad), int(accumulate), ws.data_ptr(), ws.numel()), 'tcow_gemm_tn', lib)
    return dW


def tn_group_max():
    return int(L.lib().tcow_gemm_tn_group_max())


def gemm_tn_grouped(mode, problems):
    n = len(problems)
    arr = (L.TnProblem * n)()
    for i, (dY, X, dW, db) in enumerate(problems):
        _need_cuda(dY, X, dW)
        arr[i] = L.TnProblem(dY.shape[0], dY.shape[1], X.shape[1], dY.data_ptr(), dY.stride(0), X.data_ptr(), X.stride(0), dW.data_ptr(), dW.stride(0), _p(db), 0)
    lib, dm = _sel(mode)
    ws = workspace(lib.tcow_gemm_tn_grouped_workspace_bytes(dm, n, arr), problems[0][0].device, 'tn')
    L.check(lib.tcow_gemm_tn_grouped(_stream(), dm, n, arr, ws.data_ptr(), ws.numel()), 'tcow_gemm_tn_grouped', lib)


def sgemm_batched(problems, accumulate=False):
    n = len(problems)
    arr = (L.SGemm * n)()
    for i, (A, B, C) in enumerate(problems):
        _need_cuda(A, B, C)
        M, K = A.shape
        N = B.shape[1]
        assert B.shape[0] == K and C.shape == (M, N) and C.stride(1) == 1 and A.dtype == B.dtype == C.dtype == torch.float32
        arr[i] = L.SGemm(M, N, K, A.data_ptr(), A.stride(0), A.stride(1), B.data_ptr(), B.stride(1), B.stride(0), C.data_ptr(), C.stride(0), 1 if accumulate else 0)
    L.check(L.lib().tcow_sgemm_x3_batched(_stream(), n, arr), 'tcow_sgemm_x3_batched')


def layernorm_fwd(mode, x, gamma, beta, out, mean=None, rstd=None, eps=1e-6):
    rows, D = x.shape
    lib, dm = _sel(mode)
    L.check(lib.tcow_layernorm_fwd(_stream(), dm, rows, D, x.data_ptr(), x.stride(0), gamma.data_ptr(), beta.data_ptr(), eps,
                                       out.data_ptr(), out.stride(0), _p(mean), _p(rstd)), 'tcow_layernorm_fwd', lib)
    return out


def layernorm_bwd(mode, dy, x, mean, rstd, gamma, dres, dx, dgamma=None, dbeta=None, accumulate=False, dx_cast=None, cast_scale=None,
                  colsum_out=None, colsum_scale=None, defer=None):
    rows, D = x.shape
    lib, dm = _sel(mode)
    if defer is not None and dgamma is not None:
        ws = workspace(lib.tcow_layernorm_bwd_workspace_bytes(D), x.device, 'ln_defer%d' % len(defer))
        defer.append((lib, ws, int(lib.tcow_layernorm_bwd_parts(rows, 1 if colsum_out is not None else 0)), D, dgamma, dbeta, colsum_out, bool(accumulate)))
        accumulate = int(accumulate) | 2
    else:
        ws = workspace(lib.tcow_layernorm_bwd_workspace_bytes(D), x.device, 'ln')
    L.check(lib.tcow_layernorm_bwd(_stream(), dm, rows, D, dy.data_ptr(), dy.stride(0), x.data_ptr(), x.stride(0), mean.data_ptr(),
                                   rstd.data_ptr(), gamma.data_ptr(), _p(dres), dres.stride(0) if dres is not None else 0, dx.data_ptr(),
                                   dx.stride(0), _p(dgamma), _p(dbeta), int(accumulate), ws.data_ptr(), ws.numel(),
                                   _p(dx_cast), dx_cast.stride(0) if dx_cast is not None else 0, _p(cast_scale), _p(colsum_scale), _p(colsum_out)), 'tcow_layernorm_bwd', lib)
    return dx


def layernorm_fold(jobs):
    for c0 in range(0, len(jobs), 16):
        chunk = jobs[c0:c0 + 16]
        lib = chunk[0][0]
        arr = (L.LnFoldJob * len(chunk))()
        for i, (_, ws, parts, D, dg, db, cs, acc) in enumerate(chunk):
            arr[i] = L.LnFoldJob(ws.data_ptr(), parts, D, dg.data_ptr(), db.data_ptr(), _p(cs), 1 if acc else 0)
        L.check(lib.tcow_layernorm_fold(_stream(), len(chunk), arr), 'tcow_layernorm_fold', lib)
    jobs.clear()


def attn_shape(mode, B, T, S, D, heads, causal):
    lib, dm = _sel(mode)
    sh = L.AttnShape(B, T, S, D, heads, int(causal), dm)
    sh.tcow_lib = lib
    return sh


def attn_fwd(shape, spatial, qkv, out, lse=None):
    lib = shape.tcow_lib
    fn = lib.tcow_attn_spatial_fwd if spatial else lib.tcow_attn_temporal_fwd
    L.check(fn(_stream(), ctypes.byref(shape), qkv.data_ptr(), out.data_ptr(), _p(lse)), 'tcow_attn_fwd', lib)
    return out


def attn_bwd(shape, spatial, qkv, out, dout, lse, dqkv):
    lib = shape.tcow_lib
    ws = workspace(lib.tcow_attn_bwd_workspace_bytes(ctypes.byref(shape)), qkv.device, 'attn')
    fn = lib.tcow_attn_spatial_bwd if spatial else lib.tcow_attn_temporal_bwd
    L.check(fn(_stream(), ctypes.byref(shape), qkv.data_ptr(), out.data_ptr(), dout.data_ptr(), lse.data_ptr(), dqkv.data_ptr(),
               ws.data_ptr(), ws.numel()), 'tcow_attn_bwd', lib)
    return dqkv


def attn_temporal_cached(mode, B, c, S, D, heads, causal, T_total, t0_dev, qkv, k_cache, v_cache, out):
    _need_cuda(qkv, k_cache, v_cache, out, t0_dev)
    lib, dm = _sel(mode)
    sh = L.AttnShape(B, c, S, D, heads, int(causal), F32 if dm == F32X3 else dm)
    L.check(lib.tcow_attn_temporal_cached_fwd(_stream(), ctypes.byref(sh), int(T_total), t0_dev.data_ptr(), qkv.data_ptr(), k_cache.data_ptr(),
                                              v_cache.data_ptr(), out.data_ptr()), 'tcow_attn_temporal_cached_fwd', lib)
    return out


def cls_stream(x, B, c, S, cls_cache, t0_dev):
    L.check(L.lib().tcow_cls_stream(_stream(), B, c, S, x.shape[1], x.data_ptr(), cls_cache.data_ptr(), t0_dev.data_ptr()), 'tcow_cls_stream')
    return x


def im2col(mode, rgb, query, P, pretrained_norm, out):
    B, _, T, H, W = rgb.shape
    L.check(_sel(mode)[0].tcow_im2col(_stream(), _sel(mode)[1], B, T, H, W, P, rgb.data_ptr(), query.data_ptr(), int(pretrained_norm), out.data_ptr()), 'tcow_im2col', _sel(mode)[0])
    return out


def gather_frames(frames, frame_idx, src_y, src_x):
    _need_cuda(frames, frame_idx, src_y, src_x)
    if frames.element_size() not in (1, 4) or not frames.is_contiguous():
        raise L.TcowError('gather_frames: contiguous tensor of 1- or 4-byte elements expected')
    for t in (frame_idx, src_y, src_x):
        if t.dtype != torch.int32 or not t.is_contiguous():
            raise L.TcowError('gather_frames: index tables must be contiguous int32 tensors')
    C, Tv, H, W = frames.shape
    out = torch.empty(C, frame_idx.numel(), src_y.numel(), src_x.numel(), dtype=frames.dtype, device=frames.device)
    L.check(L.lib().tcow_gather_frames(_stream(), frames.element_size(), C, Tv, H, W, frame_idx.numel(), src_y.numel(), src_x.numel(), frames.data_ptr(),
                                       frame_idx.data_ptr(), src_y.data_ptr(), src_x.data_ptr(), out.data_ptr()), 'tcow_gather_frames')
    return out


def resize_aa(frames, frame_idx, ys, xs, ymin, ysize, wy, ky, xmin, xsize, wx, kx, out_h, out_w):
    _need_cuda(frames, frame_idx, ys, xs, ymin, ysize, wy, xmin, xsize, wx)
    if frames.dtype != torch.float32 or not frames.is_contiguous():
        raise L.TcowError('resize_aa: contiguous f32 frames expected')
    for t, dt in ((frame_idx, torch.int32), (ys, torch.int32), (xs, torch.int32), (ymin, torch.int32), (ysize, torch.int32), (xmin, torch.int32), (xsize, torch.int32),
                  (wy, torch.float32), (wx, torch.float32)):
        if t.dtype != dt or not t.is_contiguous():
            raise L.TcowError('resize_aa: tables must be contiguous int32 / float32 tensors')
    C, Tv, H, W = frames.shape
    out = torch.empty(C, frame_idx.numel(), out_h, out_w, dtype=torch.float32, device=frames.device)
    L.check(L.lib().tcow_resize_aa(_stream(), C, Tv, H, W, frame_idx.numel(), ys.numel(), xs.numel(), out_h, out_w, frames.data_ptr(), frame_idx.data_ptr(), ys.data_ptr(),
                                   xs.data_ptr(), ymin.data_ptr(), ysize.data_ptr(), wy.data_ptr(), int(ky), xmin.data_ptr(), xsize.data_ptr(), wx.data_ptr(), int(kx),
                                   out.data_ptr()), 'tcow_resize_aa')
    return out


def photometric(frames, frame_idx, rect, order, factors, taps, gray):
    import ctypes
    _need_cuda(frames, frame_idx)
    if frames.dtype != torch.float32 or not frames.is_contiguous() or frames.dim() != 4 or frames.shape[0] != 3:
        raise L.TcowError('photometric: contiguous (3, Tv, H, W) f32 frames expected')
    if frame_idx.dtype != torch.int32 or not frame_idx.is_contiguous():
        raise L.TcowError('photometric: frame_idx must be a contiguous int32 tensor')
    _, Tv, H, W = frames.shape
    y0, x0, h, w = (int(v) for v in rect)
    Tc = frame_idx.numel()
    lib = L.lib()
    nb = lib.tcow_photometric_workspace_bytes(Tc)
    ws = torch.empty(max(nb // 4, 1), dtype=torch.float32, device=frames.device)
    out = torch.empty(3, Tc, h, w, dtype=torch.float32, device=frames.device)
    ops_arr = (ctypes.c_int * 4)(*([int(o) for o in order] + [0] * (4 - len(order))))
    taps_arr = (ctypes.c_float * 5)(*([float(t) for t in taps] if taps is not None else [0.0] * 5))
    fb, fc, fs, fh = (float(v) for v in factors)
    L.check(lib.tcow_photometric(_stream(), Tv, H, W, Tc, y0, x0, h, w, frames.data_ptr(), frame_idx.data_ptr(), len(order), ops_arr, fb, fc, fs, fh,
                                 1 if taps is not None else 0, taps_arr, 1 if gray else 0, ws.data_ptr(), nb, out.data_ptr()), 'tcow_photometric')
    return out


def im2col_channels(mode, src, P, normalise, out):
    B, C, T, H, W = src.shape
    L.check(_sel(mode)[0].tcow_im2col_channels(_stream(), _sel(mode)[1], B, T, H, W, P, C, src.data_ptr(), int(normalise), out.data_ptr()), 'tcow_im2col_channels', _sel(mode)[0])
    return out


def embed_fwd(x, B, T, S, cls, pos, time_embed):
    L.check(L.lib().tcow_embed_fwd(_stream(), B, T, S, x.shape[1], x.data_ptr(), cls.data_ptr(), pos.data_ptr(), time_embed.data_ptr()), 'tcow_embed_fwd')
    return x


def embed_bwd(g, B, T, S, dpos, dtime, accumulate=False):
    L.check(L.lib().tcow_embed_bwd(_stream(), B, T, S, g.shape[1], g.data_ptr(), dpos.data_ptr(), dtime.data_ptr(), int(accumulate)), 'tcow_embed_bwd')


def cls_merge(x, B, T, S, mode, backward=False, cast_mode=None, cast_out=None, cast_scale=None):
    if cast_out is not None:
        lib, dm = _sel(cast_mode)
        L.check(lib.tcow_cls_merge_bwd_cast(_stream(), dm, B, T, S, x.shape[1], x.data_ptr(), mode, cast_out.data_ptr(), cast_out.stride(0), _p(cast_scale)), 'tcow_cls_merge_bwd_cast', lib)
        return x
    L.check(L.lib().tcow_cls_merge(_stream(), B, T, S, x.shape[1], x.data_ptr(), mode, int(backward)), 'tcow_cls_merge')
    return x


def unpatchify_pool_fwd(mode, pm, BT, Hp, Wp, P, C, st, pooled):
    L.check(_sel(mode)[0].tcow_unpatchify_pool_fwd(_stream(), _sel(mode)[1], BT, Hp, Wp, P, C, st, pm.data_ptr(), pooled.data_ptr()), 'tcow_unpatchify_pool_fwd', _sel(mode)[0])
    return pooled


def unpatchify_pool_bwd(mode, dpooled, BT, Hp, Wp, P, C, st, dpm):
    L.check(_sel(mode)[0].tcow_unpatchify_pool_bwd(_stream(), _sel(mode)[1], BT, Hp, Wp, P, C, st, dpooled.data_ptr(), dpm.data_ptr()), 'tcow_unpatchify_pool_bwd', _sel(mode)[0])
    return dpm


def upsample_fwd(pooled, B, T, C, h, w, st, bilinear, out):
    L.check(L.lib().tcow_upsample_fwd(_stream(), B, T, C, h, w, st, int(bilinear), pooled.data_ptr(), out.data_ptr()), 'tcow_upsample_fwd')
    return out


def upsample_bwd(dout, B, T, C, h, w, st, bilinear, dpooled):
    L.check(L.lib().tcow_upsample_bwd(_stream(), B, T, C, h, w, st, int(bilinear), dout.data_ptr(), dpooled.data_ptr()), 'tcow_upsample_bwd')
    return dpooled


AMAX_SLOTS = 64


def upsample_bwd_amax(dout, B, T, C, h, w, st, dpooled):
    bits = torch.zeros(AMAX_SLOTS, dtype=torch.int32, device=dout.device)
    L.check(L.lib().tcow_upsample_bwd_amax(_stream(), B, T, C, h, w, st, dout.data_ptr(), dpooled.data_ptr(), bits.data_ptr(), AMAX_SLOTS), 'tcow_upsample_bwd_amax')
    return dpooled, bits.view(torch.float32).amax()


def flags_fwd(x, BT, S, Wf, bf, flags):
    L.check(L.lib().tcow_flags_fwd(_stream(), BT, S, x.shape[1], Wf.shape[0], x.data_ptr(), Wf.data_ptr(), bf.data_ptr(), flags.data_ptr()), 'tcow_flags_fwd')
    return flags


def scale_unless_one(x, scale):
    _need_cuda(x, scale)
    if x.dtype != torch.float32 or not x.is_contiguous() or scale.dtype != torch.float32 or scale.numel() != 1:
        raise L.TcowError('scale_unless_one: a contiguous f32 tensor and a one-element f32 scale')
    L.check(L.lib().tcow_scale_unless_one(_stream(), x.data_ptr(), x.numel(), scale.data_ptr()), 'tcow_scale_unless_one')
    return x


def scale_cast(mode, src, row_scale, dst):
    rows, D = src.shape
    L.check(_sel(mode)[0].tcow_scale_cast(_stream(), _sel(mode)[1], rows, D, src.data_ptr(), src.stride(0), _p(row_scale), dst.data_ptr(), dst.stride(0)), 'tcow_scale_cast', _sel(mode)[0])
    return dst


def droppath_rows(u, keep_p, mask0, B, T, S):
    _need_cuda(u, keep_p, mask0)
    depth = u.shape[0]
    if u.shape[1] != B * (S - 1) + B * T + B or u.dtype != torch.float32 or not u.is_contiguous() or mask0.numel() != B * T * S:
        raise L.TcowError('droppath_rows: u must be contiguous f32 (depth, B*(S-1) + B*T + B), mask0 [B*T*S]')
    out = torch.empty(4, depth, B * T * S, dtype=torch.float32, device=u.device)
    L.check(L.lib().tcow_droppath_rows(_stream(), depth, B, T, S, u.data_ptr(), keep_p.data_ptr(), mask0.data_ptr(), out.data_ptr()), 'tcow_droppath_rows')
    return out


def cast_transpose(mode, W, Wc=None, Wt=None):
    N, K = W.shape
    L.check(_sel(mode)[0].tcow_cast_transpose(_stream(), _sel(mode)[1], N, K, W.data_ptr(), _p(Wc), _p(Wt)), 'tcow_cast_transpose', _sel(mode)[0])


def cast_transpose_batched(mode, table, n, total_tiles):
    L.check(_sel(mode)[0].tcow_cast_transpose_batched(_stream(), _sel(mode)[1], table.data_ptr(), int(n), int(total_tiles)), 'tcow_cast_transpose_batched', _sel(mode)[0])


def mask_loss(logits, target, channel, pixel_w=None, frame_w=None, weighted_aot=False, aot_loss=0.8, topk_frac=1.0,
              loss_weight=1.0, loss_out=None, total=None, dlogits=None, focal=False):
    _need_cuda(logits, target, pixel_w, frame_w, loss_out, total, dlogits)
    BQ, C, T, H, W = logits.shape
    for t in (logits, target, dlogits):
        if t is not None and (t.dtype != torch.float32 or not t.is_contiguous() or t.shape != logits.shape):
            raise L.TcowError('mask_loss: logits / target / dlogits must be contiguous f32 tensors of one shape')
    n_frames, frame_len = BQ * T, H * W
    if pixel_w is not None and (pixel_w.dtype != torch.float32 or not pixel_w.is_contiguous() or pixel_w.numel() != n_frames * frame_len):
        raise L.TcowError('mask_loss: pixel_w must be a contiguous f32 tensor with one weight per pixel')
    if frame_w is not None and (frame_w.dtype != torch.float32 or not frame_w.is_contiguous() or frame_w.numel() != n_frames):
        raise L.TcowError('mask_loss: frame_w must be a contiguous f32 tensor with one weight per frame')
    lib = L.lib()
    nb = lib.tcow_mask_loss_workspace_bytes_for(n_frames, frame_len, float(topk_frac), float(aot_loss))
    ws = workspace(nb, logits.device, 'mask_loss')
    off = channel * T * frame_len * 4
    a = L.MaskLossArgs(n_frames, frame_len, T, logits.data_ptr() + off, C * T * frame_len, target.data_ptr() + off, C * T * frame_len,
                       _p(pixel_w), _p(frame_w), 1 if weighted_aot else 0, float(aot_loss), float(topk_frac), float(loss_weight),
                       loss_out.data_ptr(), _p(total), (dlogits.data_ptr() + off) if dlogits is not None else None,
                       C * T * frame_len, ws.data_ptr(), ws.numel(), 1 if focal else 0)
    L.check(lib.tcow_mask_loss(_stream(), ctypes.byref(a)), 'tcow_mask_loss')
    return loss_out


def mask_loss_channels(logits, target, jobs, aot_loss=0.8, topk_frac=1.0, total=None, dlogits=None, focal=False):
    _need_cuda(logits, target, total, dlogits)
    BQ, C, T, H, W = logits.shape
    for t in (logits, target, dlogits):
        if t is not None and (t.dtype != torch.float32 or not t.is_contiguous() or t.shape != logits.shape):
            raise L.TcowError('mask_loss: logits / target / dlogits must be contiguous f32 tensors of one shape')
    n_frames, frame_len = BQ * T, H * W
    lib = L.lib()
    nb = lib.tcow_mask_loss_workspace_bytes_for(n_frames, frame_len, float(topk_frac), float(aot_loss))
    arr = (L.MaskLossArgs * len(jobs))()
    for i, (channel, pixel_w, frame_w, weighted_aot, loss_weight, loss_out) in enumerate(jobs):
        _need_cuda(pixel_w, frame_w, loss_out)
        if pixel_w is not None and (pixel_w.dtype != torch.float32 or not pixel_w.is_contiguous() or pixel_w.numel() != n_frames * frame_len):
            raise L.TcowError('mask_loss: pixel_w must be a contiguous f32 tensor with one weight per pixel')
        if frame_w is not None and (frame_w.dtype != torch.float32 or not frame_w.is_contiguous() or frame_w.numel() != n_frames):
            raise L.TcowError('mask_loss: frame_w must be a contiguous f32 tensor with one weight per frame')
        ws = workspace(nb, logits.device, 'mask_loss%d' % i)
        off = channel * T * frame_len * 4
        arr[i] = L.MaskLossArgs(n_frames, frame_len, T, logits.data_ptr() + off, C * T * frame_len, target.data_ptr() + off, C * T * frame_len,
                                _p(pixel_w), _p(frame_w), 1 if weighted_aot else 0, float(aot_loss), float(topk_frac), float(loss_weight),
                                loss_out.data_ptr(), _p(total), (dlogits.data_ptr() + off) if dlogits is not None else None,
                                C * T * frame_len, ws.data_ptr(), ws.numel(), 1 if focal else 0)
    L.check(lib.tcow_mask_loss_batch(_stream(), arr, len(jobs)), 'tcow_mask_loss_batch')


def iou_counts(logits, target):
    _need_cuda(logits, target)
    if logits.shape != target.shape or logits.dtype != torch.float32 or target.dtype != torch.float32:
        raise L.TcowError('iou_counts: logits and target must be f32 tensors of one shape')
    lo = logits.contiguous(); tg = target.contiguous()
    frame_len = lo.shape[-1] * lo.shape[-2]
    out = torch.empty(lo.shape[:-2] + (3,), dtype=torch.int32, device=lo.device)
    L.check(L.lib().tcow_iou_counts(_stream(), lo.data_ptr(), tg.data_ptr(), lo.numel() // frame_len, frame_len, out.data_ptr()), 'tcow_iou_counts')
    return out


def build_masks(segm, div_segm, query_idx, front_idx, cont_idx, query_time):
    _need_cuda(segm, div_segm, query_idx, front_idx, cont_idx)
    B, _, T, H, W = segm.shape
    M = div_segm.shape[1]; Q = query_idx.shape[1]
    if segm.dtype != torch.uint8 or div_segm.dtype != torch.uint8 or not segm.is_contiguous() or not div_segm.is_contiguous():
        raise L.TcowError('build_masks: segmentation maps must be contiguous uint8 tensors')
    dev = segm.device
    qm = torch.empty(B, Q, 1, T, H, W, dtype=torch.float32, device=dev); tg = torch.empty(B, Q, 3, T, H, W, dtype=torch.float32, device=dev)
    pt = torch.empty(B, Q, 1, T, H, W, dtype=torch.uint8, device=dev); counts = torch.empty(1 + 2 * Q, dtype=torch.int32, device=dev)
    qi = query_idx.to(torch.int32).contiguous(); fi = front_idx.to(torch.int32).contiguous(); ci = cont_idx.to(torch.int32).contiguous()
    L.check(L.lib().tcow_build_masks(_stream(), B, Q, M, T, H * W, int(query_time), segm.data_ptr(), div_segm.data_ptr(), qi.data_ptr(), fi.data_ptr(),
                                     ci.data_ptr(), qm.data_ptr(), tg.data_ptr(), pt.data_ptr(), counts.data_ptr()), 'tcow_build_masks')
    return qm, tg, pt, counts


def build_query_masks(segm, div_segm, occl_fracs, dag, sel, query_time, front_occl_thres, outer_cont_thres, occluded_weight, occl_cont_zero_weight):
    _need_cuda(segm, div_segm, occl_fracs, dag, sel)
    B, _, T, H, W = segm.shape
    M = div_segm.shape[1]; K = occl_fracs.shape[1]; Q = sel.shape[1]
    if segm.dtype != torch.uint8 or div_segm.dtype != torch.uint8 or not segm.is_contiguous() or not div_segm.is_contiguous():
        raise L.TcowError('build_query_masks: segmentation maps must be contiguous uint8 tensors')
    if tuple(dag.shape) != (B, T, M, M, 3) or tuple(occl_fracs.shape[2:]) != (T, 3) or sel.dtype != torch.int64:
        raise L.TcowError('build_query_masks: occl_fracs (B,K,T,3), dag (B,T,M,M,3) and int64 sel (B,Q) expected')
    dev = segm.device
    of = occl_fracs.to(torch.float32).contiguous(); dg = dag.to(torch.float32).contiguous(); sl = sel.contiguous()
    n = B * Q * T
    qm = torch.empty(B, Q, 1, T, H, W, dtype=torch.float32, device=dev); tg = torch.empty(B, Q, 3, T, H, W, dtype=torch.float32, device=dev)
    pt = torch.empty(B, Q, 1, T, H, W, dtype=torch.uint8, device=dev); counts = torch.empty(1 + 2 * Q, dtype=torch.int32, device=dev)
    idx = torch.empty(B * Q + 2 * n, dtype=torch.int32, device=dev)
    ids = torch.empty(B, Q, T, 2, dtype=torch.uint8, device=dev)
    fl = torch.empty(2, B, Q, T, 3, dtype=torch.float32, device=dev)
    fw = torch.empty(3, B, Q, T, dtype=torch.float32, device=dev)
    f32 = np.float32
    z = f32(occl_cont_zero_weight)
    has_w = f32(f32(1.0 - occl_cont_zero_weight) + z)
    L.check(L.lib().tcow_build_query_masks(_stream(), B, Q, K, M, T, H * W, int(query_time), segm.data_ptr(), div_segm.data_ptr(), of.data_ptr(), dg.data_ptr(),
                                           sl.data_ptr(), float(f32(front_occl_thres)), float(f32(front_occl_thres / 2.0)), float(f32(outer_cont_thres)),
                                           float(f32(float(occluded_weight))), float(z), float(has_w), idx.data_ptr(), ids.data_ptr(), fl[0].data_ptr(),
                                           fl[1].data_ptr(), fw.data_ptr(), qm.data_ptr(), tg.data_ptr(), pt.data_ptr(), counts.data_ptr()),
            'tcow_build_query_masks')
    return {'query_mask': qm, 'target': tg, 'snitch_occl_by_ptr': pt, 'counts': counts, 'ids': ids, 'flags': fl[0], 'sel_occl_fracs': fl[1], 'frame_w': fw,
            'front_idx': idx[B * Q:B * Q + n].view(B, Q, T), 'cont_idx': idx[B * Q + n:].view(B, Q, T)}


def iou_means(counts):
    _need_cuda(counts)
    if counts.dtype != torch.int32 or counts.dim() != 4 or counts.shape[-1] != 3 or not counts.is_contiguous():
        raise L.TcowError('iou_means: contiguous int32 (n_seq, C, T, 3) counts expected')
    n_seq, C, T, _ = counts.shape
    out = torch.empty(12, dtype=torch.float32, device=counts.device)
    cnt = out[6:].view(torch.int32)
    L.check(L.lib().tcow_iou_means(_stream(), counts.data_ptr(), n_seq, C, T, out.data_ptr(), cnt.data_ptr()), 'tcow_iou_means')
    return out[:6], cnt


def snitch_weights(target, snitch_occl_by_ptr, frame_w, pos_count, class_balancing=True, hard_negative_factor=3.0):
    _need_cuda(target, snitch_occl_by_ptr, frame_w, pos_count)
    B, Q, C, T, H, W = target.shape
    if not target.is_contiguous() or not snitch_occl_by_ptr.is_contiguous() or target.dtype != torch.float32 or snitch_occl_by_ptr.dtype != torch.uint8:
        raise L.TcowError('snitch_weights: target must be contiguous f32 and snitch_occl_by_ptr contiguous u8')
    out = torch.empty(B, Q, T, H, W, dtype=torch.float32, device=target.device)
    fw = frame_w.to(torch.float32).contiguous()
    lib = L.lib()
    ws = workspace(lib.tcow_snitch_weights_workspace_bytes(B * Q * T, H, W), target.device, 'snitch_w')
    L.check(lib.tcow_snitch_weights(_stream(), B * Q, T, H, W, target.data_ptr(), C * T * H * W, snitch_occl_by_ptr.data_ptr(), fw.data_ptr(), pos_count.data_ptr(),
                                    1 if class_balancing else 0, float(hard_negative_factor), out.data_ptr(), ws.data_ptr(), ws.numel()), 'tcow_snitch_weights')
    return out
```

### tcow_amd/optim.py

```python
import weakref

import numpy as np
import torch

from . import _lib as L

CHUNK = 65536


def _ops_stream():
    from .ops import _stream
    return _stream()


class FusedAdamWClip(torch.optim.Optimizer):
    def __init__(self, params, lr=1e-4, betas=(0.9, 0.999), eps=1e-8, weight_decay=0.01, max_norm=0.3, module=None, fuse_cast=True):
        super().__init__(params, dict(lr=lr, betas=betas, eps=eps, weight_decay=weight_decay))
        if len(self.param_groups) != 1:
            raise L.TcowError('FusedAdamWClip takes one parameter group (train.py:239-241 builds exactly one)')
        self.max_norm = max_norm
        self._table = None
        self._key = None
        self.scratch = None
        self.on_step = []
        self._tracker = None
        self._skip_carry = 0.0
        self._live = []; self._seen_grads = []; self._step_base = 0; self._steps_pending = 0
        self.fuse_cast = bool(fuse_cast)
        self._tiles = None; self._flat_table = None; self._cast_keys = frozenset(); self._wreg_gen = None
        if module is not None:
            tracker = getattr(module, 'seeker', module)
            self._tracker = tracker
            if hasattr(tracker, 'invalidate_weight_cache'):
                self.on_step.append(tracker.invalidate_weight_cache)
            tracker.__dict__['_optim_ref'] = weakref.ref(self)
        assert L.lib().tcow_adamw_chunk_bytes() == 40

    @property
    def params(self):
        return self.param_groups[0]['params']

    @property
    def lr(self):
        return self.param_groups[0]['lr']

    @property
    def step_count(self):
        self._flush_steps()
        for p in self.params:
            st = self.state.get(p)
            if st:
                return int(st['step'])
        return 0

    def _flush_steps(self):
        if self._steps_pending and self._live:
            torch._foreach_add_([self.state[p]['step'] for p in self._live], float(self._steps_pending))
            self._step_base += self._steps_pending
        self._steps_pending = 0

    def _cast_registry(self):
        trk = self._tracker
        if not self.fuse_cast or trk is None or getattr(trk, 'precision', None) not in ('bf16', 'fp16') or getattr(trk, '_is_replica', False):
            return {}
        out = {}
        for k, (p, Wc, Wt, N, K) in (trk.__dict__.get('_wreg') or {}).items():
            if isinstance(k, int) and isinstance(p, torch.nn.Parameter) and Wc is not None and Wt is not None and N % 64 == 0 and K % 64 == 0 and p.numel() == N * K:
                out[id(p)] = (Wc, Wt, N, K)
        return out

    def _lib(self):
        trk = self._tracker
        return L.lib('fp16') if (trk is not None and getattr(trk, 'precision', None) == 'fp16' and self._tiles is not None) else L.lib()

    def _build(self, live):
        reg = self._cast_registry()
        fused = [p for p in live if id(p) in reg]
        rows, flat_rows = [], []
        for p in live:
            st = self.state[p]
            if 'exp_avg' not in st:
                st['step'] = torch.tensor(0.0, dtype=torch.float32)
                st['exp_avg'] = torch.zeros_like(p, dtype=torch.float32, memory_format=torch.preserve_format)
                st['exp_avg_sq'] = torch.zeros_like(p, dtype=torch.float32, memory_format=torch.preserve_format)
            m, v = st['exp_avg'], st['exp_avg_sq']
            g = p.grad
            if not (p.is_contiguous() and g.is_contiguous() and m.is_contiguous() and v.is_contiguous() and p.dtype == torch.float32 and g.dtype == torch.float32
                    and m.dtype == torch.float32 and v.dtype == torch.float32):
                raise L.TcowError('FusedAdamWClip needs contiguous f32 parameters, gradients and moments')
            n = p.numel()
            for off in range(0, n, CHUNK):
                rows.append((p.data_ptr() + 4 * off, g.data_ptr() + 4 * off, m.data_ptr() + 4 * off, v.data_ptr() + 4 * off, min(CHUNK, n - off)))
                if id(p) not in reg:
                    flat_rows.append(rows[-1])
        if self.scratch is not None:
            self._skip_carry += float(self.scratch[-1])
        self._table = torch.from_numpy(np.asarray(rows, dtype=np.int64)).to(live[0].device)
        self.scratch = torch.zeros(len(rows) + 3, dtype=torch.float32, device=live[0].device)
        self.scratch[-1] = self._skip_carry
        self._tiles = None; self._flat_table = None; self._cast_keys = frozenset()
        trk = self._tracker
        self._wreg_gen = trk.__dict__.get('_wreg_gen') if trk is not None else None
        if fused:
            assert L.lib().tcow_adamw_tile_bytes() == 56
            recs = []
            for p in fused:
                Wc, Wt, N, K = reg[id(p)]
                st = self.state[p]
                n0, k0 = np.meshgrid(np.arange(0, N, 64, dtype=np.int64), np.arange(0, K, 64, dtype=np.int64), indexing='ij')
                o = (n0 * K + k0).reshape(-1); ot = (k0 * N + n0).reshape(-1)
                r = np.empty((o.size, 7), dtype=np.int64)
                r[:, 0] = p.data_ptr() + 4 * o; r[:, 1] = p.grad.data_ptr() + 4 * o; r[:, 2] = st['exp_avg'].data_ptr() + 4 * o; r[:, 3] = st['exp_avg_sq'].data_ptr() + 4 * o
                r[:, 4] = Wc.data_ptr() + 2 * o; r[:, 5] = Wt.data_ptr() + 2 * ot; r[:, 6] = K | (N << 32)
                recs.append(r)
            self._tiles = torch.from_numpy(np.concatenate(recs, axis=0)).to(live[0].device)
            self._flat_table = torch.from_numpy(np.asarray(flat_rows, dtype=np.int64).reshape(-1, 5)).to(live[0].device)
            self._cast_keys = frozenset(id(p) for p in fused)

    @torch.no_grad()
    def step(self, closure=None):
        loss = None
        if closure is not None:
            with torch.enable_grad():
                loss = closure()
        grp = self.param_groups[0]
        params = grp['params']
        fast = self._key is not None and len(params) == len(self._seen_grads)
        if fast:
            for p, g in zip(params, self._seen_grads):
                if p.grad is not g:
                    fast = False
                    break
        if fast and self._live:
            fast = self._live[0].grad.data_ptr() == self._key[0][1] and self._live[-1].grad.data_ptr() == self._key[-1][1]
        if fast and self._tracker is not None and self.fuse_cast:
            fast = self._tracker.__dict__.get('_wreg_gen') == self._wreg_gen
        if fast:
            live = self._live
        else:
            live = [p for p in params if p.grad is not None]
            if not live:
                return loss
            self._flush_steps()
            key = tuple((id(p), p.grad.data_ptr(), self.state[p]['exp_avg'].data_ptr() if 'exp_avg' in self.state[p] else 0) for p in live)
            gen = self._tracker.__dict__.get('_wreg_gen') if self._tracker is not None else None
            if key != self._key or (self.fuse_cast and gen != self._wreg_gen):
                self._build(live)
                self._key = tuple((id(p), p.grad.data_ptr(), self.state[p]['exp_avg'].data_ptr()) for p in live)
            self._live = live
            self._seen_grads = [p.grad for p in params]
            self._step_base = int(self.state[live[0]]['step'])
            self._steps_pending = 0
        if not live:
            return loss
        step = self._step_base + self._steps_pending + 1
        trk = self._tracker
        inv_scale = trk.__dict__.get('pending_inv_scale') if trk is not None else None
        if self._tiles is not None:
            lib = self._lib()
            L.check(lib.tcow_adamw_clip_step_cast(_ops_stream(), self._table.data_ptr(), self._table.shape[0], self._flat_table.data_ptr() if self._flat_table.shape[0] else None,
                                                  self._flat_table.shape[0], self._tiles.data_ptr(), self._tiles.shape[0],
                                                  float(grp['lr']), float(grp['betas'][0]), float(grp['betas'][1]), float(grp['eps']), float(grp['weight_decay']), step,
                                                  float(self.max_norm or 0.0), self.scratch.data_ptr(), inv_scale.data_ptr() if inv_scale is not None else None),
                    'tcow_adamw_clip_step_cast', lib)
            trk.__dict__['_opt_cast_keys'] = self._cast_keys
        else:
            L.check(L.lib().tcow_adamw_clip_step_scaled(_ops_stream(), self._table.data_ptr(), self._table.shape[0], float(grp['lr']),
                                                        float(grp['betas'][0]), float(grp['betas'][1]), float(grp['eps']), float(grp['weight_decay']), step,
                                                        float(self.max_norm or 0.0), self.scratch.data_ptr(), inv_scale.data_ptr() if inv_scale is not None else None),
                    'tcow_adamw_clip_step_scaled')
        ls = getattr(trk, 'ls_log2', None) if trk is not None and getattr(trk, 'precision', None) == 'fp16' and getattr(trk, 'loss_scale', None) == 'dynamic' else None
        if ls is not None and ls.device == self.scratch.device:
            ok = self.scratch[-3] >= 0
            ls.copy_(torch.minimum(ls + torch.where(ok, 1.0 / 256.0, -4.0), torch.full_like(ls, -2.0)))
        self._steps_pending += 1
        torch.autograd.graph.increment_version(live)
        for cb in self.on_step:
            cb()
        return loss

    def unscale_(self):
        trk = self._tracker
        inv = trk.__dict__.get('pending_inv_scale') if trk is not None else None
        if inv is None:
            return
        seen = set()
        for p in self.params:
            if p.grad is not None and p.grad.data_ptr() not in seen:
                seen.add(p.grad.data_ptr())
                p.grad.mul_(inv)
        trk.__dict__['pending_inv_scale'] = None

    def detach(self):
        trk = self._tracker
        if trk is not None:
            self.unscale_()
            ref = trk.__dict__.get('_optim_ref')
            if ref is not None and ref() is self:
                trk.__dict__.pop('_optim_ref', None)

    def grad_norm(self):
        return self.scratch[-2]

    @property
    def skipped_steps(self):
        return None if self.scratch is None else self.scratch[-1]

    def state_dict(self):
        self._flush_steps()
        sd = super().state_dict()
        skipped = float(self.scratch[-1]) if self.scratch is not None else 0.0
        if skipped:
            sd['state'] = {k: dict(st) for k, st in sd['state'].items()}
            for st in sd['state'].values():
                if 'step' in st:
                    st['step'] = st['step'] - skipped
        return sd

    def load_state_dict(self, sd):
        self._steps_pending = 0
        super().load_state_dict(sd)
        self._key = None; self._live = []; self._seen_grads = []
        self._skip_carry = 0.0
        self.scratch = None
```

### tcow_amd/seeker.py

```python
import math
from functools import partial

import torch
import torch.nn as nn

from . import ops
from ._lib import TcowError

TIMESFORMER_MEAN = 0.45
TIMESFORMER_STD = 0.225



def _trunc_normal_(t, std=.02):
    with torch.no_grad():
        return nn.init.trunc_normal_(t, mean=0., std=std, a=-2., b=2.)


class _Attention(nn.Module):
    def __init__(self, dim):
        super().__init__()
        self.qkv = nn.Linear(dim, dim * 3, bias=True)
        self.proj = nn.Linear(dim, dim)


class _Mlp(nn.Module):
    def __init__(self, dim, hidden):
        super().__init__()
        self.fc1 = nn.Linear(dim, hidden)
        self.fc2 = nn.Linear(hidden, dim)


class _Block(nn.Module):
    def __init__(self, dim, mlp_ratio, divided=True):
        super().__init__()
        self.norm1 = nn.LayerNorm(dim, eps=1e-6)
        self.attn = _Attention(dim)
        if divided:
            self.temporal_norm1 = nn.LayerNorm(dim, eps=1e-6)
            self.temporal_attn = _Attention(dim)
            self.temporal_fc = nn.Linear(dim, dim)
        self.norm2 = nn.LayerNorm(dim, eps=1e-6)
        self.mlp = _Mlp(dim, int(dim * mlp_ratio))


class _PatchEmbed(nn.Module):
    def __init__(self, patch, in_chans, dim):
        super().__init__()
        self.proj = nn.Conv2d(in_chans, dim, kernel_size=patch, stride=patch)


class _VisionTransformer(nn.Module):
    def __init__(self, img_size, patch, in_chans, dim, depth, mlp_ratio, num_frames, divided=True):
        super().__init__()
        self.embed_dim = dim
        self.patch_embed = _PatchEmbed(patch, in_chans, dim)
        n_patches = (img_size[0] // patch) * (img_size[1] // patch)
        self.cls_token = nn.Parameter(torch.zeros(1, 1, dim))
        self.pos_embed = nn.Parameter(torch.zeros(1, n_patches + 1, dim))
        self.time_embed = nn.Parameter(torch.zeros(1, num_frames, dim))
        self.blocks = nn.ModuleList([_Block(dim, mlp_ratio, divided) for _ in range(depth)])
        self.norm = nn.LayerNorm(dim, eps=1e-6)
        _trunc_normal_(self.pos_embed)
        _trunc_normal_(self.cls_token)
        for m in self.modules():
            if isinstance(m, nn.Linear):
                _trunc_normal_(m.weight)
                nn.init.constant_(m.bias, 0)
            elif isinstance(m, nn.LayerNorm):
                nn.init.constant_(m.bias, 0)
                nn.init.constant_(m.weight, 1.0)
        for blk in self.blocks if divided else []:
            nn.init.constant_(blk.temporal_fc.weight, 0)
            nn.init.constant_(blk.temporal_fc.bias, 0)


class _TimeSformer(nn.Module):
    def __init__(self, **kw):
        super().__init__()
        self.model = _VisionTransformer(**kw)


class _Backbone(nn.Module):
    def __init__(self, **kw):
        super().__init__()
        self.timesformer = _TimeSformer(**kw)
        self.output_feature_dim = self.timesformer.model.embed_dim


_DEPTH_GEOMETRY = {12: (768, 12), 18: (896, 14), 24: (1024, 16)}



class QueryMaskTracker(nn.Module):

    def __init__(self, logger, num_total_frames=24, num_visible_frames=16, frame_height=224, frame_width=288,
                 tracker_pretrained=False, attention_type='divided_space_time', patch_size=16, causal_attention=False,
                 norm_embeddings=False, drop_path_rate=0.1, network_depth=12, track_map_stride=4,
                 track_map_resize='bilinear', query_channels=1, output_channels=3, flag_channels=3,
                 embed_dim=None, num_heads=None, precision='bf16'):
        super().__init__()
        self.logger = logger
        self.num_total_frames = num_total_frames
        self.num_visible_frames = num_visible_frames
        self.frame_height = frame_height
        self.frame_width = frame_width
        self.attention_type = attention_type
        self.patch_size = patch_size
        self.causal_attention = int(causal_attention)
        self.norm_embeddings = bool(norm_embeddings)
        self.drop_path_rate = drop_path_rate
        self.network_depth = network_depth
        self.track_map_stride = track_map_stride
        self.track_map_resize = track_map_resize
        self.query_channels = query_channels
        self.output_channels = output_channels
        self.flag_channels = flag_channels
        self.input_channels = 3 + query_channels
        self.set_precision(precision)

        from .checkpoint import parse_tracker_pretrained
        self.tracker_pretrained, self.pretrained_path = parse_tracker_pretrained(tracker_pretrained)
        if logger is not None:
            logger.info(f'(QueryMaskTracker) tracker_pretrained: {self.tracker_pretrained} '
                        f'pretrained_path: {self.pretrained_path}')

        assert attention_type in ['divided_space_time', 'space_only', 'joint_space_time']
        if attention_type == 'space_only':
            raise TcowError("attention_type='space_only' is not runnable through Seeker (vision_tf.py:127 needs time_embed, vit.py:263-265)")
        if query_channels != 1:
            raise TcowError('query_channels must be 1 (mask_tracker.py:105)')
        if embed_dim is None or num_heads is None:
            if network_depth not in _DEPTH_GEOMETRY:
                raise ValueError(f'Invalid network depth {network_depth}, must be one of 12, 18, 24.')
            embed_dim, num_heads = _DEPTH_GEOMETRY[network_depth]
        if embed_dim != num_heads * 64:
            raise TcowError(f'head_dim must be 64 (embed_dim={embed_dim}, num_heads={num_heads})')
        self.embed_dim, self.num_heads = embed_dim, num_heads
        assert frame_height % patch_size == 0
        assert frame_width % patch_size == 0
        if track_map_stride > 1 and patch_size % track_map_stride != 0:
            raise TcowError('track_map_stride must divide patch_size')
        if track_map_resize not in ('bilinear', 'nearest'):
            raise TcowError(f'unsupported track_map_resize {track_map_resize}')

        self.tracker_backbone = _Backbone(img_size=(frame_height, frame_width), patch=patch_size,
                                          in_chans=self.input_channels, dim=embed_dim, depth=network_depth,
                                          mlp_ratio=4, num_frames=num_total_frames, divided=(attention_type == 'divided_space_time'))
        self.use_feature_dim = embed_dim
        self.tracker_post_linear = nn.Linear(embed_dim, output_channels * patch_size * patch_size)
        if flag_channels > 0:
            self.flag_post_linear = nn.Linear(embed_dim, flag_channels)
        if self.tracker_pretrained:
            from .checkpoint import load_pretrained_vit
            load_pretrained_vit(self, self.pretrained_path, logger)
        self._wcache = {}
        self._gbufs = {}
        self.register_buffer('ls_log2', torch.full((), -2.0, dtype=torch.float32), persistent=False)
        self.persistent_grads = False
        self.forced_drop_masks = None
        self.grad_hook = None

    def set_precision(self, precision):
        if precision not in ('bf16', 'fp16', 'fp32', 'bf16x3'):
            raise ValueError("precision must be 'bf16', 'fp16', 'fp32' or 'bf16x3'")
        self.precision = precision
        self.mode = ops.BF16 if precision == 'bf16' else ops.FP16 if precision == 'fp16' else ops.F32
        if 'ls_log2' in self._buffers:
            with torch.no_grad():
                self.ls_log2.fill_(-2.0)
        self.loss_scale = 'dynamic'
        self.gemm_mode = ops.F32X3 if precision == 'bf16x3' else self.mode
        self._wcache = {}
        self.__dict__.pop('_wreg', None); self.__dict__.pop('_wtab', None); self.__dict__.pop('_foldreg', None)
        self.__dict__['_wreg_gen'] = self.__dict__.get('_wreg_gen', 0) + 1
        return self

    def invalidate_weight_cache(self):
        self._wepoch = getattr(self, '_wepoch', 0) + 1
        if self.__dict__.get('_wreg'):
            from . import engine
            engine.refresh_weights(self)

    def _drop_operand_caches(self):
        self._wcache = {}
        self.__dict__.pop('_wreg', None); self.__dict__.pop('_wtab', None); self.__dict__.pop('_foldreg', None)
        self.__dict__['_wreg_gen'] = self.__dict__.get('_wreg_gen', 0) + 1
        self._gbufs = {}

    def _apply(self, fn, *a, **kw):
        self._drop_operand_caches()
        self.invalidate_param_cache()
        return super()._apply(fn, *a, **kw)

    @property
    def vit(self):
        return self.tracker_backbone.timesformer.model

    def geometry(self, B, T=None):
        P = self.patch_size
        Hp, Wp = self.frame_height // P, self.frame_width // P
        N = Hp * Wp
        T = self.num_total_frames if T is None else T
        return dict(B=B, T=T, Hp=Hp, Wp=Wp, N=N, S=N + 1, D=self.embed_dim, heads=self.num_heads, P=P, M=B * T * (N + 1))

    def stream(self, batch_size=1, queries_per_clip=1, graph=False):
        from .stream import SeekerStream
        return SeekerStream(self, batch_size, queries_per_clip, graph)

    def param_list(self):
        cached = self.__dict__.get('_param_list_cache')
        if cached is not None and cached[0] is self.vit.cls_token and cached[-1] is (self.flag_post_linear if self.flag_channels > 0 else self.tracker_post_linear).bias:
            return cached
        ps = self._param_list_uncached()
        self.__dict__['_param_list_cache'] = ps
        return ps

    def invalidate_param_cache(self):
        self.__dict__.pop('_param_list_cache', None)

    def _param_list_uncached(self):
        v = self.vit
        ps = [v.cls_token, v.pos_embed, v.time_embed, v.patch_embed.proj.weight, v.patch_embed.proj.bias]
        for b in v.blocks:
            if self.attention_type == 'divided_space_time':
                ps += [b.temporal_norm1.weight, b.temporal_norm1.bias, b.temporal_attn.qkv.weight, b.temporal_attn.qkv.bias,
                       b.temporal_attn.proj.weight, b.temporal_attn.proj.bias, b.temporal_fc.weight, b.temporal_fc.bias]
            ps += [b.norm1.weight, b.norm1.bias, b.attn.qkv.weight, b.attn.qkv.bias, b.attn.proj.weight, b.attn.proj.bias,
                   b.norm2.weight, b.norm2.bias, b.mlp.fc1.weight, b.mlp.fc1.bias, b.mlp.fc2.weight, b.mlp.fc2.bias]
        ps += [v.norm.weight, v.norm.bias, self.tracker_post_linear.weight, self.tracker_post_linear.bias]
        if self.flag_channels > 0:
            ps += [self.flag_post_linear.weight, self.flag_post_linear.bias]
        return ps

    def forward(self, input_frames, query_mask):
        (B, _, T, Hf, Wf) = input_frames.shape
        assert query_mask.shape[1] == 1
        assert query_mask.shape[0] % B == 0 and query_mask.shape[2:] == input_frames.shape[2:]
        assert T == self.num_total_frames
        assert Hf == self.frame_height and Wf == self.frame_width
        assert self.attention_type == 'divided_space_time' or self.causal_attention == 0
        if not input_frames.is_cuda:
            raise TcowError('Seeker (tcow_amd) runs on the GPU only: move inputs and module to cuda')
        if query_mask.device != input_frames.device or self.vit.pos_embed.device != input_frames.device:
            raise TcowError(f'Seeker (tcow_amd): inputs ({input_frames.device}, {query_mask.device}) and parameters ({self.vit.pos_embed.device}) must share one device')
        if getattr(self, '_is_replica', False):
            self._wcache, self._gbufs = {}, {}
            self.__dict__.pop('_wreg', None); self.__dict__.pop('_wtab', None); self.__dict__.pop('_foldreg', None)
            self.__dict__['_wreg_gen'] = self.__dict__.get('_wreg_gen', 0) + 1
        rgb = input_frames.to(torch.float32).contiguous()
        qm = query_mask.to(torch.float32).contiguous()
        from .engine import SeekerFunction
        with torch.cuda.device(input_frames.device):
            out_mask, out_flags = SeekerFunction.apply(self, rgb, qm, *self.param_list())
        if self.flag_channels <= 0:
            out_flags = None
        return (out_mask, out_flags)


class Seeker(nn.Module):

    shares_rgb = True

    def __init__(self, logger, **kwargs):
        super().__init__()
        self.logger = logger
        self.seeker_args = {k: v for k, v in kwargs.items() if k != 'precision'}
        self.seeker = QueryMaskTracker(logger, **kwargs)

    def forward(self, *args):
        return self.seeker(*args)

    def stream(self, batch_size=1, queries_per_clip=1, graph=False):
        return self.seeker.stream(batch_size, queries_per_clip, graph)
```

Measured before the change: 36.79 clips/s.

## Batch fold-product sgemms into one cached mixed launch and pair AdamW cast tiles

Adds a mixed batched bf16x3 sgemm kernel. It handles heterogeneous problems in a single launch, takes an optional rank-1 update term computed with MFMA in the epilogue, and caches the device record table per tag. Forward and backward temporal fold products now use it in place of several chunked batched sgemm and TN launches. Separately, the AdamW cast kernel now processes two adjacent weight tiles per block to cut block count and per-tile overhead. The risks are more register pressure in the mixed kernel, stale cached records if pointers change, and extra code paths.

```diff
diff --git a/include/tcow_hip.h b/include/tcow_hip.h
--- a/include/tcow_hip.h
+++ b/include/tcow_hip.h
@@ -20,7 +20,7 @@
 #define TCOW_ACT_GELU_DSAVE 3
 #define TCOW_ACT_MUL_AUX 4
 
-#define TCOW_ABI_VERSION 11
+#define TCOW_ABI_VERSION 12
 int tcow_version(void);
 const char* tcow_last_error(void);
 
@@ -71,6 +71,16 @@
     int accumulate;
 } tcow_sgemm;
 int tcow_sgemm_x3_batched(void* stream, int n, const tcow_sgemm* problems);
+typedef struct {
+    int M, N, K;
+    const float* A; long sai, sak;
+    const float* B; long sbj, sbk;
+    float* C; long ldc;
+    const float* r1u; const float* r1v;
+} tcow_sgemm_mixed;
+long tcow_sgemm_x3_mixed_record_bytes(void);
+int tcow_sgemm_x3_mixed_prepare(int n, const tcow_sgemm_mixed* problems, void* host_records, int* launch);
+int tcow_sgemm_x3_mixed_launch(void* stream, int n, const void* dev_records, int launch0, int launch1);
 
 int tcow_layernorm_fwd(void* stream, int dtype, int rows, int D, const float* x, long ldx, const float* gamma,
                        const float* beta, float eps, void* y, long ldy, float* mean, float* rstd);
@@ -160,6 +170,8 @@
 long tcow_adamw_tile_bytes(void);
 int tcow_adamw_clip_step_cast(void* stream, const void* chunks, int n_chunks, const void* flat_chunks, int n_flat, const void* tiles, int n_tiles, float lr, float beta1,
                               float beta2, float eps, float weight_decay, int step, float max_norm, float* scratch, const float* grad_inv_scale);
+int tcow_adamw_clip_step_cast_runs(void* stream, const void* chunks, int n_chunks, const void* flat_chunks, int n_flat, const void* tiles, int n_tiles, float lr, float beta1,
+                                   float beta2, float eps, float weight_decay, int step, float max_norm, float* scratch, const float* grad_inv_scale, int run);
 
 typedef struct {
     long n_frames, frame_len, frames_per_seq;
diff --git a/tcow_amd/_lib.py b/tcow_amd/_lib.py
--- a/tcow_amd/_lib.py
+++ b/tcow_amd/_lib.py
@@ -32,6 +32,13 @@
                 ('A', ctypes.c_void_p), ('sai', ctypes.c_long), ('sak', ctypes.c_long),
                 ('B', ctypes.c_void_p), ('sbj', ctypes.c_long), ('sbk', ctypes.c_long),
                 ('C', ctypes.c_void_p), ('ldc', ctypes.c_long), ('accumulate', ctypes.c_int)]
+
+
+class SGemmMixed(ctypes.Structure):
+    _fields_ = [('M', ctypes.c_int), ('N', ctypes.c_int), ('K', ctypes.c_int),
+                ('A', ctypes.c_void_p), ('sai', ctypes.c_long), ('sak', ctypes.c_long),
+                ('B', ctypes.c_void_p), ('sbj', ctypes.c_long), ('sbk', ctypes.c_long),
+                ('C', ctypes.c_void_p), ('ldc', ctypes.c_long), ('r1u', ctypes.c_void_p), ('r1v', ctypes.c_void_p)]
 
 
 class TnProblem(ctypes.Structure):
@@ -74,6 +81,9 @@
     'tcow_gemm_tn_grouped': (_i, [_vp, _i, _i, _vp, _vp, _l]),
     'tcow_gemm_tn_group_max': (_i, []),
     'tcow_sgemm_x3_batched': (_i, [_vp, _i, _vp]),
+    'tcow_sgemm_x3_mixed_record_bytes': (_l, []),
+    'tcow_sgemm_x3_mixed_prepare': (_i, [_i, _vp, _vp, ctypes.POINTER(ctypes.c_int)]),
+    'tcow_sgemm_x3_mixed_launch': (_i, [_vp, _i, _vp, _i, _i]),
     'tcow_layernorm_fwd': (_i, [_vp, _i, _i, _i, _vp, _l, _vp, _vp, _f, _vp, _l, _vp, _vp]),
     'tcow_layernorm_bwd_workspace_bytes': (_l, [_i]),
     'tcow_layernorm_bwd': (_i, [_vp, _i, _i, _i, _vp, _l, _vp, _l, _vp, _vp, _vp, _vp, _l, _vp, _l, _vp, _vp, _i, _vp, _l, _vp, _l, _vp, _vp, _vp]),
@@ -114,6 +124,7 @@
     'tcow_adamw_clip_step_scaled': (_i, [_vp, _vp, _i, _f, _f, _f, _f, _f, _i, _f, _vp, _vp]),
     'tcow_adamw_tile_bytes': (_l, []),
     'tcow_adamw_clip_step_cast': (_i, [_vp, _vp, _i, _vp, _i, _vp, _i, _f, _f, _f, _f, _f, _i, _f, _vp, _vp]),
+    'tcow_adamw_clip_step_cast_runs': (_i, [_vp, _vp, _i, _vp, _i, _vp, _i, _f, _f, _f, _f, _f, _i, _f, _vp, _vp, _i]),
     'tcow_mask_loss_workspace_bytes': (ctypes.c_size_t, [_l, _l]),
     'tcow_mask_loss_workspace_bytes_for': (ctypes.c_size_t, [_l, _l, ctypes.c_double, _f]),
     'tcow_mask_loss': (_i, [_vp, ctypes.POINTER(MaskLossArgs)]),
@@ -127,7 +138,7 @@
 }
 
 
-ABI_VERSION = 11
+ABI_VERSION = 12
 
 
 def _declare(L, tolerant=False):
diff --git a/tcow_amd/csrc/gemm_x3.hip b/tcow_amd/csrc/gemm_x3.hip
--- a/tcow_amd/csrc/gemm_x3.hip
+++ b/tcow_amd/csrc/gemm_x3.hip
@@ -130,7 +130,8 @@
 }
 
 template <int LDA, int LDB>
-__device__ __forceinline__ void gemm_x3_body(const F32Params& p, const int bid, const int kz, char* smem) {
+__device__ __forceinline__ void gemm_x3_body(const F32Params& p, const int bid, const int kz, char* smem, const float* __restrict__ r1u = nullptr,
+                                             const float* __restrict__ r1v = nullptr) {
     char* a_hi = smem; char* a_lo = smem + XPLANE; char* b_hi = smem + 2 * XPLANE; char* b_lo = smem + 3 * XPLANE;
     const int tid = threadIdx.x, lane = tid & 63, wave = tid >> 6;
     const int wm = wave >> 1, wn = wave & 1, l31 = lane & 31, hi = lane >> 5;
@@ -199,6 +200,32 @@
         if (gn + 1 < p.N) b4.y = p.bias[gn + 1];
         if (gn + 2 < p.N) b4.z = p.bias[gn + 2];
         if (gn + 3 < p.N) b4.w = p.bias[gn + 3];
+    }
+    if (r1u) {
+        x3_bf16x8 uh[2], ul[2], vh[2], vl[2];
+#pragma unroll
+        for (int i = 0; i < 2; ++i) {
+            const int gm = m0 + wm * 64 + i * 32 + l31, gnn = n0 + wn * 64 + i * 32 + l31;
+            const float uu = (hi == 0 && gm < p.M) ? r1u[gm] : 0.f, vv = (hi == 0 && gnn < p.N) ? r1v[gnn] : 0.f;
+            uint32_t h, l;
+            split2(uu, 0.f, h, l);
+            uh[i] = __builtin_bit_cast(x3_bf16x8, make_uint4(h, 0u, 0u, 0u)); ul[i] = __builtin_bit_cast(x3_bf16x8, make_uint4(l, 0u, 0u, 0u));
+            split2(vv, 0.f, h, l);
+            vh[i] = __builtin_bit_cast(x3_bf16x8, make_uint4(h, 0u, 0u, 0u)); vl[i] = __builtin_bit_cast(x3_bf16x8, make_uint4(l, 0u, 0u, 0u));
+        }
+#pragma unroll
+        for (int i = 0; i < 2; ++i)
+#pragma unroll
+            for (int j = 0; j < 2; ++j) {
+                f32x16 t;
+#pragma unroll
+                for (int r = 0; r < 16; ++r) t[r] = 0.f;
+                t = __builtin_amdgcn_mfma_f32_32x32x16_bf16(vh[j], ul[i], t, 0, 0, 0);
+                t = __builtin_amdgcn_mfma_f32_32x32x16_bf16(vl[j], uh[i], t, 0, 0, 0);
+                t = __builtin_amdgcn_mfma_f32_32x32x16_bf16(vh[j], uh[i], t, 0, 0, 0);
+#pragma unroll
+                for (int r = 0; r < 16; ++r) acc[i][j][r] = (t[r] + 0.f) + acc[i][j][r];
+            }
     }
     float* slab = p.slab ? p.slab + (size_t)kz * p.M * p.N : nullptr;
 #pragma unroll
@@ -245,6 +272,27 @@
     gemm_x3_body<LDA, LDB>(p, blockIdx.x, 0, smem);
 }
 
+enum { MIX_KK = 0, MIX_KR = 1, MIX_RR = 2, MIX_RK = 3 };
+struct X3MixRec { F32Params p; const float* r1u; const float* r1v; int kind; int tiles; };
+template <bool VEC>
+__global__ __launch_bounds__(256, VEC ? 3 : 2) void gemm_x3_mixed_kernel(const X3MixRec* __restrict__ recs) {
+    __shared__ __attribute__((aligned(16))) char smem[4 * XPLANE];
+    const X3MixRec* __restrict__ r = recs + blockIdx.y;
+    if ((int)blockIdx.x >= r->tiles) return;
+    const F32Params& p = r->p;
+    const float* r1u = r->r1u; const float* r1v = r->r1v;
+    if constexpr (VEC) {
+        switch (r->kind) {
+            case MIX_KK: gemm_x3_body<LD_KVEC, LD_KVEC>(p, blockIdx.x, 0, smem, r1u, r1v); break;
+            case MIX_KR: gemm_x3_body<LD_KVEC, LD_RVEC>(p, blockIdx.x, 0, smem, r1u, r1v); break;
+            case MIX_RR: gemm_x3_body<LD_RVEC, LD_RVEC>(p, blockIdx.x, 0, smem, r1u, r1v); break;
+            default: gemm_x3_body<LD_RVEC, LD_KVEC>(p, blockIdx.x, 0, smem, r1u, r1v); break;
+        }
+    } else {
+        gemm_x3_body<LD_ANY, LD_ANY>(p, blockIdx.x, 0, smem, r1u, r1v);
+    }
+}
+
 }
 
 int tcow_launch_slab_reduce(hipStream_t stream, const float* slab, int nz, long slab_stride, long rows, long cols, float* out, long ldo, int accumulate,
@@ -327,3 +375,44 @@
     TCOW_CHECK_LAUNCH();
     return TCOW_OK;
 }
+
+static int x3_loader_mixed(const float* P, long s_row, long s_k, int nrows, int K) {
+    const bool al = (reinterpret_cast<uintptr_t>(P) & 15) == 0;
+    if (s_k == 1 && al && (nrows == 1 || (s_row & 3) == 0) && (K & 3) == 0 && K >= 4) return LD_KVEC;
+    return x3_loader(P, s_row, s_k, nrows, K);
+}
+
+extern "C" long tcow_sgemm_x3_mixed_record_bytes(void) { return (long)sizeof(X3MixRec); }
+
+extern "C" int tcow_sgemm_x3_mixed_prepare(int n, const tcow_sgemm_mixed* probs, void* host_records, int* launch) {
+    TCOW_CHECK_ARG(n >= 1 && n <= 65535 && probs && host_records && launch, "tcow_sgemm_x3_mixed_prepare: 1 .. 65535 problems, non-NULL tables (got %d)", n);
+    X3MixRec* recs = (X3MixRec*)host_records;
+    int maxtiles = 0, vec = 1;
+    for (int i = 0; i < n; ++i) {
+        const tcow_sgemm_mixed& s = probs[i];
+        TCOW_CHECK_ARG(s.M > 0 && s.N > 0 && s.K > 0 && s.A && s.B && s.C && s.ldc >= s.N && (!s.r1u == !s.r1v), "tcow_sgemm_x3_mixed_prepare: bad problem %d", i);
+        X3MixRec& r = recs[i];
+        F32Params& p = r.p;
+        p.M = s.M; p.N = s.N; p.K = s.K; p.A = s.A; p.sai = s.sai; p.sak = s.sak; p.B = s.B; p.sbj = s.sbj; p.sbk = s.sbk;
+        p.C = s.C; p.ldc = s.ldc; p.bias = nullptr; p.row_scale = nullptr; p.resid = nullptr; p.ldr = 0; p.act = 0; p.aux = nullptr; p.ldaux = 0; p.bias2 = nullptr; p.row_scale2 = nullptr;
+        p.kps = ((s.K + XK - 1) / XK) * XK; p.slab = nullptr;
+        r.r1u = s.r1u; r.r1v = s.r1v;
+        const int la = x3_loader_mixed(s.A, s.sai, s.sak, s.M, s.K), lb = x3_loader_mixed(s.B, s.sbj, s.sbk, s.N, s.K);
+        if (la == LD_ANY || lb == LD_ANY) vec = 0;
+        r.kind = la == LD_KVEC ? (lb == LD_KVEC ? MIX_KK : MIX_KR) : (lb == LD_RVEC ? MIX_RR : MIX_RK);
+        r.tiles = cdiv(s.N, XT) * cdiv(s.M, XT);
+        if (r.tiles > maxtiles) maxtiles = r.tiles;
+    }
+    launch[0] = maxtiles; launch[1] = vec;
+    return TCOW_OK;
+}
+
+extern "C" int tcow_sgemm_x3_mixed_launch(void* stream, int n, const void* dev_records, int grid_x, int vec) {
+    TCOW_CHECK_ARG(n >= 1 && n <= 65535 && dev_records && grid_x >= 1, "tcow_sgemm_x3_mixed_launch: bad arguments");
+    const dim3 grid(grid_x, n);
+    hipStream_t st = (hipStream_t)stream;
+    if (vec) hipLaunchKernelGGL(gemm_x3_mixed_kernel<true>, grid, dim3(256), 0, st, (const X3MixRec*)dev_records);
+    else hipLaunchKernelGGL(gemm_x3_mixed_kernel<false>, grid, dim3(256), 0, st, (const X3MixRec*)dev_records);
+    TCOW_CHECK_LAUNCH();
+    return TCOW_OK;
+}
diff --git a/tcow_amd/csrc/optim.hip b/tcow_amd/csrc/optim.hip
--- a/tcow_amd/csrc/optim.hip
+++ b/tcow_amd/csrc/optim.hip
@@ -99,6 +99,84 @@
     }
 }
 
+typedef uint32_t tcow_u32x2 __attribute__((ext_vector_type(2)));
+template <int NR>
+__device__ __forceinline__ void adamw_cast_run(const CastTile& d, uint32_t* __restrict__ lds, float coef, float decay, float step_size, float beta1, float beta2,
+                                               float bc2_sqrt, float eps) {
+    constexpr int LPR = 16 * NR, RPP = 256 / LPR, PITCH = 32 * NR + 1;
+    auto upd = [&](float& p, float g, float& m, float& v) {
+        g *= coef;
+        p *= decay;
+        m = beta1 * m + (1.0f - beta1) * g;
+        v = beta2 * v + (1.0f - beta2) * g * g;
+        p -= step_size * m / (sqrtf(v) / bc2_sqrt + eps);
+    };
+    GLB_PTR(float) gp = (GLB_PTR(float))d.p; GLB_PTR(float) gm = (GLB_PTR(float))d.m; GLB_PTR(float) gv = (GLB_PTR(float))d.v;
+    GLB_PTR(const float) gg = (GLB_PTR(const float))d.g;
+    GLB_PTR(bf16_t) gwc = (GLB_PTR(bf16_t))d.wc; GLB_PTR(bf16_t) gwt = (GLB_PTR(bf16_t))d.wt;
+    const int c4 = ((int)threadIdx.x % LPR) * 4, r0 = (int)threadIdx.x / LPR;
+#pragma unroll 1
+    for (int b = 0; b < NR; ++b) {
+        f32x4 p[4], m[4], v[4], g[4];
+#pragma unroll
+        for (int i = 0; i < 4; ++i) {
+            const uint32_t o = (uint32_t)((r0 + RPP * (4 * b + i)) * d.K + c4);
+            p[i] = *reinterpret_cast<GLB_PTR(const f32x4)>(gp + o); m[i] = *reinterpret_cast<GLB_PTR(const f32x4)>(gm + o);
+            v[i] = *reinterpret_cast<GLB_PTR(const f32x4)>(gv + o); g[i] = *reinterpret_cast<GLB_PTR(const f32x4)>(gg + o);
+        }
+#pragma unroll
+        for (int i = 0; i < 4; ++i) {
+            const int r = r0 + RPP * (4 * b + i);
+            const uint32_t o = (uint32_t)(r * d.K + c4);
+#pragma unroll
+            for (int e = 0; e < 4; ++e) { float pe = p[i][e], me = m[i][e], ve = v[i][e]; upd(pe, g[i][e], me, ve); p[i][e] = pe; m[i][e] = me; v[i][e] = ve; }
+            *reinterpret_cast<GLB_PTR(f32x4)>(gp + o) = p[i]; *reinterpret_cast<GLB_PTR(f32x4)>(gm + o) = m[i]; *reinterpret_cast<GLB_PTR(f32x4)>(gv + o) = v[i];
+            const uint32_t w0 = pack_bf2(p[i][0], p[i][1]), w1 = pack_bf2(p[i][2], p[i][3]);
+            *reinterpret_cast<GLB_PTR(tcow_u32x2)>(gwc + o) = (tcow_u32x2){w0, w1};
+            lds[r * PITCH + (c4 >> 1)] = w0; lds[r * PITCH + (c4 >> 1) + 1] = w1;
+        }
+    }
+    __syncthreads();
+    const int nn = threadIdx.x & 7, kq = threadIdx.x >> 3;
+#pragma unroll
+    for (int ps = 0; ps < 2 * NR; ++ps) {
+        const int k = kq + 32 * ps, sh = (k & 1) * 16;
+        uint32_t h[8];
+#pragma unroll
+        for (int j = 0; j < 8; ++j) h[j] = (lds[(nn * 8 + j) * PITCH + (k >> 1)] >> sh) & 0xffffu;
+        *reinterpret_cast<GLB_PTR(tcow_u32x4)>(gwt + (size_t)k * d.N + nn * 8) = (tcow_u32x4){h[0] | (h[1] << 16), h[2] | (h[3] << 16), h[4] | (h[5] << 16), h[6] | (h[7] << 16)};
+    }
+}
+
+template <int RUN>
+__global__ __launch_bounds__(256, 3) void adamw_cast_run_kernel(const CastTile* __restrict__ tiles, int n_tiles, const float* __restrict__ coef_ptr, float lr, float beta1,
+                                                             float beta2, float eps, float weight_decay, int step) {
+    __shared__ uint32_t lds[64 * (32 * RUN + 1)];
+    const float coef = coef_ptr[0];
+    if (coef < 0.f) return;
+    const float eff = fmaxf((float)step - coef_ptr[2], 1.0f);
+    const float bc1 = 1.0f - powf(beta1, eff), bc2_sqrt = sqrtf(1.0f - powf(beta2, eff));
+    const float decay = 1.0f - lr * weight_decay, step_size = lr / bc1;
+    const int t0 = blockIdx.x * RUN;
+    const int cnt = n_tiles - t0 < RUN ? n_tiles - t0 : RUN;
+    const CastTile d = tiles[t0];
+    bool adj = cnt == RUN;
+    for (int j = 1; j < RUN && adj; ++j) {
+        const CastTile e = tiles[t0 + j];
+        adj = e.K == d.K && e.N == d.N && e.p == d.p + 64 * j && e.g == d.g + 64 * j && e.m == d.m + 64 * j && e.v == d.v + 64 * j && e.wc == d.wc + 64 * j &&
+              e.wt == d.wt + (size_t)64 * j * d.N;
+    }
+    if (adj) {
+        adamw_cast_run<RUN>(d, lds, coef, decay, step_size, beta1, beta2, bc2_sqrt, eps);
+    } else {
+        for (int j = 0; j < cnt; ++j) {
+            const CastTile e = tiles[t0 + j];
+            adamw_cast_run<1>(e, lds, coef, decay, step_size, beta1, beta2, bc2_sqrt, eps);
+            __syncthreads();
+        }
+    }
+}
+
 }
 
 extern "C" {
@@ -106,10 +184,10 @@
 long tcow_adamw_chunk_bytes(void) { return (long)sizeof(Chunk); }
 long tcow_adamw_tile_bytes(void) { return (long)sizeof(CastTile); }
 
-int tcow_adamw_clip_step_cast(void* stream, const void* chunks, int n_chunks, const void* flat_chunks, int n_flat, const void* tiles, int n_tiles, float lr, float beta1,
-                              float beta2, float eps, float weight_decay, int step, float max_norm, float* scratch, const float* grad_inv_scale) {
-    TCOW_CHECK_ARG(chunks && scratch && n_chunks > 0 && step >= 1 && n_flat >= 0 && (flat_chunks || n_flat == 0) && n_tiles >= 0 && (tiles || n_tiles == 0),
-                   "tcow_adamw_clip_step_cast: bad arguments");
+int tcow_adamw_clip_step_cast_runs(void* stream, const void* chunks, int n_chunks, const void* flat_chunks, int n_flat, const void* tiles, int n_tiles, float lr, float beta1,
+                                   float beta2, float eps, float weight_decay, int step, float max_norm, float* scratch, const float* grad_inv_scale, int run) {
+    TCOW_CHECK_ARG(chunks && scratch && n_chunks > 0 && step >= 1 && n_flat >= 0 && (flat_chunks || n_flat == 0) && n_tiles >= 0 && (tiles || n_tiles == 0) &&
+                   (run == 1 || run == 2), "tcow_adamw_clip_step_cast_runs: bad arguments");
     const Chunk* c = (const Chunk*)chunks;
     hipLaunchKernelGGL(sumsq_kernel, dim3(n_chunks), dim3(256), 0, (hipStream_t)stream, c, scratch);
     TCOW_CHECK_LAUNCH();
@@ -120,10 +198,18 @@
         TCOW_CHECK_LAUNCH();
     }
     if (n_tiles > 0) {
-        hipLaunchKernelGGL(adamw_cast_kernel, dim3(n_tiles), dim3(256), 0, (hipStream_t)stream, (const CastTile*)tiles, scratch + n_chunks, lr, beta1, beta2, eps, weight_decay, step);
+        const CastTile* t = (const CastTile*)tiles;
+        if (run == 2) hipLaunchKernelGGL(adamw_cast_run_kernel<2>, dim3(cdiv(n_tiles, 2)), dim3(256), 0, (hipStream_t)stream, t, n_tiles, scratch + n_chunks, lr, beta1, beta2, eps, weight_decay, step);
+        else hipLaunchKernelGGL(adamw_cast_kernel, dim3(n_tiles), dim3(256), 0, (hipStream_t)stream, t, scratch + n_chunks, lr, beta1, beta2, eps, weight_decay, step);
         TCOW_CHECK_LAUNCH();
     }
     return TCOW_OK;
+}
+
+int tcow_adamw_clip_step_cast(void* stream, const void* chunks, int n_chunks, const void* flat_chunks, int n_flat, const void* tiles, int n_tiles, float lr, float beta1,
+                              float beta2, float eps, float weight_decay, int step, float max_norm, float* scratch, const float* grad_inv_scale) {
+    return tcow_adamw_clip_step_cast_runs(stream, chunks, n_chunks, flat_chunks, n_flat, tiles, n_tiles, lr, beta1, beta2, eps, weight_decay, step, max_norm, scratch,
+                                          grad_inv_scale, 1);
 }
 
 int tcow_adamw_clip_step_scaled(void* stream, const void* chunks, int n_chunks, float lr, float beta1, float beta2, float eps, float weight_decay, int step,
diff --git a/tcow_amd/engine.py b/tcow_amd/engine.py
--- a/tcow_amd/engine.py
+++ b/tcow_amd/engine.py
@@ -70,7 +70,12 @@
     return ops.is16(module.mode) and module.attention_type == 'divided_space_time'
 
 
-def _fold_products(ents):
+def _fold_products(ents, module=None):
+    if module is not None and module.__dict__.get('_mixed_fold', True):
+        ops.sgemm_mixed([(e['fc'].detach(), e['proj'].detach(), e['W32']) for e in ents] +
+                        [(e['fc'].detach(), e['bproj'].detach().view(1, -1).t(), e['b32'].view(-1, 1)) for e in ents],
+                        cache=module.__dict__.setdefault('_foldtab', {}), tag='fwd')
+        return
     for c0 in range(0, len(ents), 24):
         ops.sgemm_batched([(e['fc'].detach(), e['proj'].detach(), e['W32']) for e in ents[c0:c0 + 24]])
         ops.sgemm_batched([(e['fc'].detach(), e['bproj'].detach().view(1, -1).t(), e['b32'].view(-1, 1)) for e in ents[c0:c0 + 24]])
@@ -111,7 +116,7 @@
     if folds:
         live = [ent for k, ent in folds.items() if k in reg]
         if live:
-            _fold_products(live)
+            _fold_products(live, module)
     done = module.__dict__.pop('_opt_cast_keys', None) or ()
     all_ents = list(reg.items())
     ents = [(k, v) for k, v in all_ents if k not in done]
@@ -546,6 +551,21 @@
 
     def finish_fold_group():
         if not fold_jobs:
+            return
+        if module.__dict__.get('_mixed_fold', True):
+            probs = []
+            for (i, tW, tb) in fold_jobs:
+                o_ = 5 + i * BP
+                probs.append((params[o_ + ix['tfc']].detach().t(), tW, grads[o_ + ix['tproj']]))
+            for (i, tW, tb) in fold_jobs:
+                o_ = 5 + i * BP
+                wfc, wp, bp = params[o_ + ix['tfc']].detach(), params[o_ + ix['tproj']].detach(), params[o_ + ix['tproj'] + 1].detach()
+                probs.append((tW, wp.t(), grads[o_ + ix['tfc']], tb, bp))
+            for (i, tW, tb) in fold_jobs:
+                o_ = 5 + i * BP
+                probs.append((params[o_ + ix['tfc']].detach().t(), tb.view(-1, 1), grads[o_ + ix['tproj'] + 1].view(-1, 1)))
+            ops.sgemm_mixed(probs, cache=module.__dict__.setdefault('_foldtab', {}), tag='bwd')
+            fold_jobs.clear()
             return
         nt_, r1_, tn_, gv_ = [], [], [], []
         for (i, tW, tb) in fold_jobs:
diff --git a/tcow_amd/ops.py b/tcow_amd/ops.py
--- a/tcow_amd/ops.py
+++ b/tcow_amd/ops.py
@@ -111,6 +111,37 @@
         assert B.shape[0] == K and C.shape == (M, N) and C.stride(1) == 1 and A.dtype == B.dtype == C.dtype == torch.float32
         arr[i] = L.SGemm(M, N, K, A.data_ptr(), A.stride(0), A.stride(1), B.data_ptr(), B.stride(1), B.stride(0), C.data_ptr(), C.stride(0), 1 if accumulate else 0)
     L.check(L.lib().tcow_sgemm_x3_batched(_stream(), n, arr), 'tcow_sgemm_x3_batched')
+
+
+def sgemm_mixed(problems, cache=None, tag=None):
+    key = []
+    for pr in problems:
+        for t in pr:
+            key.append(None if t is None else (t.data_ptr(), t.shape, t.stride()))
+    dev = problems[0][2].device
+    key = (tuple(key), str(dev))
+    ent = cache.get(tag) if cache is not None else None
+    lib = L.lib()
+    n = len(problems)
+    if ent is None or ent[0] != key:
+        arr = (L.SGemmMixed * n)()
+        for i, pr in enumerate(problems):
+            A, B, C = pr[:3]
+            u, v = (pr[3], pr[4]) if len(pr) > 3 else (None, None)
+            _need_cuda(A, B, C, u, v)
+            M, K = A.shape
+            N = B.shape[1]
+            assert B.shape[0] == K and C.shape == (M, N) and C.stride(1) == 1 and A.dtype == B.dtype == C.dtype == torch.float32
+            if u is not None:
+                assert u.dtype == v.dtype == torch.float32 and u.numel() == M and v.numel() == N and u.is_contiguous() and v.is_contiguous()
+            arr[i] = L.SGemmMixed(M, N, K, A.data_ptr(), A.stride(0), A.stride(1), B.data_ptr(), B.stride(1), B.stride(0), C.data_ptr(), C.stride(0), _p(u), _p(v))
+        host = torch.empty(n * int(lib.tcow_sgemm_x3_mixed_record_bytes()), dtype=torch.uint8).pin_memory()
+        launch = (ctypes.c_int * 2)()
+        L.check(lib.tcow_sgemm_x3_mixed_prepare(n, arr, host.data_ptr(), launch), 'tcow_sgemm_x3_mixed_prepare')
+        ent = (key, host.to(dev, non_blocking=True), int(launch[0]), int(launch[1]), host)
+        if cache is not None:
+            cache[tag] = ent
+    L.check(lib.tcow_sgemm_x3_mixed_launch(_stream(), n, ent[1].data_ptr(), ent[2], ent[3]), 'tcow_sgemm_x3_mixed_launch')
 
 
 def layernorm_fwd(mode, x, gamma, beta, out, mean=None, rstd=None, eps=1e-6):
diff --git a/tcow_amd/optim.py b/tcow_amd/optim.py
--- a/tcow_amd/optim.py
+++ b/tcow_amd/optim.py
@@ -27,6 +27,7 @@
         self._skip_carry = 0.0
         self._live = []; self._seen_grads = []; self._step_base = 0; self._steps_pending = 0
         self.fuse_cast = bool(fuse_cast)
+        self.cast_run = 2
         self._tiles = None; self._flat_table = None; self._cast_keys = frozenset(); self._wreg_gen = None
         if module is not None:
             tracker = getattr(module, 'seeker', module)
@@ -158,11 +159,12 @@
         inv_scale = trk.__dict__.get('pending_inv_scale') if trk is not None else None
         if self._tiles is not None:
             lib = self._lib()
-            L.check(lib.tcow_adamw_clip_step_cast(_ops_stream(), self._table.data_ptr(), self._table.shape[0], self._flat_table.data_ptr() if self._flat_table.shape[0] else None,
-                                                  self._flat_table.shape[0], self._tiles.data_ptr(), self._tiles.shape[0],
-                                                  float(grp['lr']), float(grp['betas'][0]), float(grp['betas'][1]), float(grp['eps']), float(grp['weight_decay']), step,
-                                                  float(self.max_norm or 0.0), self.scratch.data_ptr(), inv_scale.data_ptr() if inv_scale is not None else None),
-                    'tcow_adamw_clip_step_cast', lib)
+            L.check(lib.tcow_adamw_clip_step_cast_runs(_ops_stream(), self._table.data_ptr(), self._table.shape[0], self._flat_table.data_ptr() if self._flat_table.shape[0] else None,
+                                                       self._flat_table.shape[0], self._tiles.data_ptr(), self._tiles.shape[0],
+                                                       float(grp['lr']), float(grp['betas'][0]), float(grp['betas'][1]), float(grp['eps']), float(grp['weight_decay']), step,
+                                                       float(self.max_norm or 0.0), self.scratch.data_ptr(), inv_scale.data_ptr() if inv_scale is not None else None,
+                                                       int(self.cast_run)),
+                    'tcow_adamw_clip_step_cast_runs', lib)
             trk.__dict__['_opt_cast_keys'] = self._cast_keys
         else:
             L.check(L.lib().tcow_adamw_clip_step_scaled(_ops_stream(), self._table.data_ptr(), self._table.shape[0], float(grp['lr']),
diff --git a/tcow_amd/seeker.py b/tcow_amd/seeker.py
--- a/tcow_amd/seeker.py
+++ b/tcow_amd/seeker.py
@@ -172,7 +172,7 @@
         self.loss_scale = 'dynamic'
         self.gemm_mode = ops.F32X3 if precision == 'bf16x3' else self.mode
         self._wcache = {}
-        self.__dict__.pop('_wreg', None); self.__dict__.pop('_wtab', None); self.__dict__.pop('_foldreg', None)
+        self.__dict__.pop('_wreg', None); self.__dict__.pop('_wtab', None); self.__dict__.pop('_foldreg', None); self.__dict__.pop('_foldtab', None)
         self.__dict__['_wreg_gen'] = self.__dict__.get('_wreg_gen', 0) + 1
         return self
 
@@ -184,7 +184,7 @@
 
     def _drop_operand_caches(self):
         self._wcache = {}
-        self.__dict__.pop('_wreg', None); self.__dict__.pop('_wtab', None); self.__dict__.pop('_foldreg', None)
+        self.__dict__.pop('_wreg', None); self.__dict__.pop('_wtab', None); self.__dict__.pop('_foldreg', None); self.__dict__.pop('_foldtab', None)
         self.__dict__['_wreg_gen'] = self.__dict__.get('_wreg_gen', 0) + 1
         self._gbufs = {}
 
@@ -246,7 +246,7 @@
             raise TcowError(f'Seeker (tcow_amd): inputs ({input_frames.device}, {query_mask.device}) and parameters ({self.vit.pos_embed.device}) must share one device')
         if getattr(self, '_is_replica', False):
             self._wcache, self._gbufs = {}, {}
-            self.__dict__.pop('_wreg', None); self.__dict__.pop('_wtab', None); self.__dict__.pop('_foldreg', None)
+            self.__dict__.pop('_wreg', None); self.__dict__.pop('_wtab', None); self.__dict__.pop('_foldreg', None); self.__dict__.pop('_foldtab', None)
             self.__dict__['_wreg_gen'] = self.__dict__.get('_wreg_gen', 0) + 1
         rgb = input_frames.to(torch.float32).contiguous()
         qm = query_mask.to(torch.float32).contiguous()
```

After: 36.95 clips/s (median of 6 runs). Within noise of the previous version (+0.4%).
